# pathint/RankCompV3.jl

Measured on AMD Instinct MI355X. Metric: gene-pair·sample comparisons/sec at 20k genes × 1k samples, higher is better.
Workload: dtype u16

## Files before the change

### rankcompv3.jl_amd/_ffi.py

```python
from __future__ import annotations

import ctypes
import os
import subprocess
from typing import NamedTuple

import numpy as np

_HERE = os.path.dirname(os.path.abspath(__file__))
LIB_PATH = os.environ.get("REO_LIB_PATH") or os.path.join(_HERE, "libreo_hip.so")
CSRC = os.path.join(_HERE, "csrc")

REO_OK, REO_EINVAL, REO_EHIP, REO_ECOMM, REO_ENOMEM = 0, -1, -2, -3, -4
NTIMINGS = 12
CALL_BINS = 8192

SYMBOLS = [
    "reo_version", "reo_last_error", "reo_create", "reo_destroy", "reo_trim_memory", "reo_set_shard", "reo_set_allreduce", "reo_set_allgather",
    "reo_create_multi", "reo_comm_unique_id", "reo_comm_init_rank",
    "reo_set_matrix_f64", "reo_set_matrix_i64", "reo_set_matrix_dev_f64", "reo_set_matrix_dev_i64",
    "reo_set_matrix_f32", "reo_set_matrix_i32", "reo_set_matrix_dev_f32", "reo_set_matrix_dev_i32",
    "reo_set_matrix_rm_f64", "reo_set_matrix_rm_i64", "reo_set_matrix_rm_f32", "reo_set_matrix_rm_i32",
    "reo_set_matrix_csc_f64", "reo_set_matrix_csc_i64", "reo_set_matrix_csc_f32", "reo_set_matrix_csc_i32",
    "reo_set_groups", "reo_compute_thresholds", "reo_set_thresholds", "reo_get_thresholds", "reo_threshold",
# ... 1058 lines not shown
        out = np.zeros((cont.shape[0], 5), dtype=np.float64)
        check(self._L.reo_mccullagh(self._h, _ptr(cont), cont.shape[0], _ptr(out)))
        return out

    @staticmethod
    def _pseudobulk_args(cells, order, chunk_ptr):
        order = np.ascontiguousarray(order, dtype=np.int32)
        chunk_ptr = np.ascontiguousarray(chunk_ptr, dtype=np.int32)
        n_out = chunk_ptr.size - 1
        if hasattr(cells, "tocsc"):
            m = cells.tocsc()
            m.sort_indices()
            G, C = m.shape
            isint = np.issubdtype(m.dtype, np.integer)
            val = np.ascontiguousarray(m.data, dtype=np.int64 if isint else np.float64)
            colptr = np.ascontiguousarray(m.indptr, dtype=np.int64)
            rowidx = np.ascontiguousarray(m.indices, dtype=np.int32)
            args = (G, C, _ptr(colptr), _ptr(rowidx), _ptr(val), _ptr(order), order.size, _ptr(chunk_ptr), n_out)
            return "csc", "i64" if isint else "f64", args, G, (m, val, colptr, rowidx, order, chunk_ptr)
        X = np.asarray(cells)
        isint = np.issubdtype(X.dtype, np.integer)
        Xf = np.asfortranarray(X, dtype=np.int64 if isint else np.float64)
        G, C = Xf.shape
        args = (_ptr(Xf), G, C, G, _ptr(order), order.size, _ptr(chunk_ptr), n_out)
        return "dense", "i64" if isint else "f64", args, G, (Xf, order, chunk_ptr)

    def pseudobulk(self, cells, order, chunk_ptr) -> np.ndarray:
        form, ty, args, G, keep = self._pseudobulk_args(cells, order, chunk_ptr)
        out = np.zeros((G, args[-1]), dtype=np.int64 if ty == "i64" else np.float64, order="F")
        check(getattr(self._L, f"reo_pseudobulk_{form}_{ty}")(self._h, *args, _ptr(out)))
        return out

    def set_matrix_pseudobulk(self, cells, order, chunk_ptr) -> None:
        if is_device_sparse(cells) or is_device_tensor(cells):
            order = np.ascontiguousarray(order, dtype=np.int32)
            chunk_ptr = np.ascontiguousarray(chunk_ptr, dtype=np.int32)
            n_out = chunk_ptr.size - 1
            tail = (_ptr(order) if order.size else None, order.size, _ptr(chunk_ptr), n_out)
            if is_device_sparse(cells):
                ty, G, C, nnz, colptr, rowidx, val, bits, keep = device_csc_entry(cells)
                check(getattr(self._L, "reo_set_matrix_pseudobulk_csc_dev_" + ty)(self._h, G, C, nnz, _dptr(colptr), _dptr(rowidx), bits, _dptr(val), *tail))
            else:
                ptr, G, C, ld, ty, keep = device_matrix(cells)
                check(getattr(self._L, "reo_set_matrix_pseudobulk_dense_dev_" + ty)(self._h, ctypes.c_void_p(ptr), G, C, ld, *tail))
            self.G, self.S = G, n_out
            return
        form, ty, args, G, keep = self._pseudobulk_args(cells, order, chunk_ptr)
        check(getattr(self._L, f"reo_set_matrix_pseudobulk_{form}_{ty}")(self._h, *args))
        self.G, self.S = G, args[-1]

    def filter_matrix(self, min_profiles: int = 0, min_features: int = 0):
        info = self.info()
        pk = np.zeros(info["S"], dtype=np.uint8)
        gk = np.zeros(info["G"], dtype=np.uint8)
        sk, gkn = ctypes.c_int64(0), ctypes.c_int64(0)
        check(self._L.reo_filter_matrix(self._h, int(min_profiles), int(min_features), _ptr(pk) if pk.size else None, _ptr(gk) if gk.size else None,
                                        ctypes.byref(sk), ctypes.byref(gkn)))
        self.G, self.S = int(gkn.value), int(sk.value)
        return pk.astype(bool), gk.astype(bool)

    def get_matrix(self) -> np.ndarray:
        info = self.info()
        dt = {1: np.float64, 2: np.int64, 3: np.float32}.get(info["resident_dtype"])
        if dt is None:
            raise DimensionMismatch(REO_EINVAL, "no expression matrix set")
        out = np.zeros((info["G"], info["S"]), dtype=dt, order="F")
        check(self._L.reo_get_matrix(self._h, _ptr(out), out.nbytes))
        return out

    def set_profiling(self, on: bool) -> None:
        check(self._L.reo_set_profiling(self._h, 1 if on else 0))

    def reset_timings(self) -> None:
        check(self._L.reo_reset_timings(self._h))

    def timings(self) -> dict:
        ms = np.zeros(NTIMINGS, dtype=np.float64)
        check(self._L.reo_get_timings(self._h, _ptr(ms), NTIMINGS))
        return {"transform_ms": ms[0], "k1_ms": ms[1], "k2_ms": ms[2], "iter_ms": ms[3], "k3_ms": max(ms[3] - ms[2], 0.0), "k2_launches": int(ms[4]),
                "k1_launches": int(ms[5]), "exchange_ms": ms[6], "pseudobulk_ms": ms[7], "k2_full_ms": ms[8],
                "k2_full_launches": int(ms[9]), "k2_delta_ms": ms[10], "set_matrix_host_wall_ms": ms[11]}

    def info(self) -> dict:
        w = np.zeros(40, dtype=np.int64)
        check(self._L.reo_get_info(self._h, _ptr(w), 40))
        v = np.zeros(28, dtype=np.int64)
        v[:] = w[:28]
        return {"G": int(v[0]), "S": int(v[1]), "Gp": int(v[2]), "table_bytes": int(v[3]), "has_ties": int(v[4]),
                "tiles_owned": int(v[5]), "tiles_total": int(v[6]), "tile_i": int(v[7]), "chunk_j": int(v[8]),
                "chunks_per_panel": int(v[9]), "unit_h": int(v[10]), "sample_slots": int(v[11]),
                "shared_group_counts": int(v[12]), "group_count_bytes": int(v[13]), "transform_in_lds": int(v[14]), "xcc_local_histograms": int(v[15]),
                "cycle_period": int(v[16]), "cycle_found_at_pass": int(v[17]), "cycle_passes_skipped": int(v[18]), "upload_link_bytes": int(v[19]),
                "eager_range_launches": int(v[20]), "rowmajor_upload": int(v[21]),
                "csc_upload": int(v[22]), "csc_nnz": int(v[23]), "resident_dtype": int(v[24]),
                "k1_slot_order": int(v[25]), "k1_half_tiles_separated": int(v[26]), "csc_device": int(v[27]),
                "k1_unslot_form": int(w[28]), "contrast_treat": int(w[29]), "k1_slot_sides": int(w[30]),
                "masked_build": int(w[31]), "k1_slot_slice": int(w[32]), "planes_on_demand": int(w[33]),
                "perm_batch": int(w[34]), "perm_kernel_us": int(w[35]),
                "top_pairs_hist_us": int(w[36]), "top_pairs_emit_us": int(w[37]),
                "top_pairs_null_batch": int(w[38]), "top_pairs_null_us": int(w[39])}
```

### rankcompv3.jl_amd/csrc/api.hip

```cpp
#include <execinfo.h>
#include <signal.h>
#include <unistd.h>

#include <ctime>
#include <algorithm>
#include <chrono>
#include <cmath>
#include <cstdarg>
#include <cstdio>
#include <cstdlib>
#include <cstring>

#include "reo_internal.h"
#include "contrast.h"
#include "masked_pairs.h"
#include "perm_null.h"
#include "sample_counts.h"
#include "upload_csc.h"

#include <mutex>
#include <unordered_map>

namespace reo {

// ... 228 lines not shown
    static bool done = false;
    if (done) return;
    done = true;
    void *warm[2];
    (void)backtrace(warm, 2);
    struct sigaction sa;
    memset(&sa, 0, sizeof sa);
    sa.sa_handler = segv_backtrace;
    sa.sa_flags = SA_NODEFER;
    sigaction(SIGSEGV, &sa, &g_old_action[0]);
    sigaction(SIGBUS, &sa, &g_old_action[1]);
    sigaction(SIGABRT, &sa, &g_old_action[2]);
}

static double wall_us()
{
    timespec ts;
    clock_gettime(CLOCK_MONOTONIC, &ts);
    return ts.tv_sec * 1e6 + ts.tv_nsec * 1e-3;
}

static void drop_ref_mask(reo_ctx *c, const char *why)
{
    c->ref_slot = -1;
    c->ref_gone = why;
}

int32_t wait_or_drop_table(reo_ctx *c)
{
    const hipError_t e = stream_wait(c);
    if (e == hipSuccess) return REO_OK;
    c->built_k = -1;
    c->table_complete = false;
    drop_ref_mask(c, "a kernel queued on this context failed and the class table was dropped");
    set_error("a kernel queued on this context failed: %s (the class table was dropped: call reo_build_pairs again)", hipGetErrorString(e));
    return REO_EHIP;
}

int32_t use(reo_ctx *c)
{
    if (!c) { set_error("null context"); return REO_EINVAL; }
    REO_HIP_CHECK(hipSetDevice(c->device));
    return REO_OK;
}

int32_t no_multi(reo_ctx *c, const char *what)
{
    if (!c) { set_error("null context"); return REO_EINVAL; }
    if (c->in_multi) {
        set_error("%s is not available on a reo_create_multi context (every device would need the matrix: use one process per GPU, each with its own context)", what);
        return REO_EINVAL;
    }
    return REO_OK;
}

bool mask_in_force(reo_ctx *c)
{
    if (c->vmask_set && (c->vmask_G != c->G || c->vmask_S != c->S)) { c->vmask_set = false; c->vwords_valid = false; }
    return c->vmask_set;
}

int32_t refuse_under_mask(reo_ctx *c, const char *what)
{
    if (!c || !mask_in_force(c)) return REO_OK;
    char msg[320];
    mp_query_refusal(what, msg, sizeof msg);
    set_error("%s", msg);
    return REO_EINVAL;
}

static void invalidate(reo_ctx *c)
{
    drop_ref_mask(c, "the matrix or the groups changed after the last reo_identify_degs (reo_set_matrix_*, reo_filter_matrix, reo_set_groups): "
                     "the class table it ran on is gone");
    c->transformed = false;
    c->planes_ready = false; c->planes_on_demand = 0; c->last_k1_slot_slice = 0;
    c->built_k = -1;
    c->built_treat = -1;
    c->built_masked = 0;
    c->gc_valid = false;
    c->eager_k1 = false;
    c->vwords_valid = false;
    (void)mask_in_force(c);
    c->last_k1_slots = 0; c->last_k1_slot_sides = 0; c->k1_slot_items = nullptr; c->k1_slot_items_n = 0; c->k1_slot_gp = 0;
}

static size_t elem_bytes(int dtype) { return dtype >= 3 ? 4 : 8; }

static int32_t check_shape(int64_t G, int64_t S)
{
    if (G < 2 || G > kMaxGenes || S < 2 || S > (1 << 20)) {
        set_error("matrix is %lld x %lld; G must be in [2, %d] and S in [2, 1048576]", (long long)G, (long long)S, kMaxGenes);
        return REO_EINVAL;
    }
    return REO_OK;
}

static int32_t set_matrix(reo_ctx *c, const void *X, int64_t G, int64_t S, int64_t ld, int dtype, bool on_device, int layout = kLayoutColMajor)
{
    const bool rowmajor = layout == kLayoutRowMajor;
    int32_t rc = use(c);
    if (rc) return rc;
    if (dtype >= 3 && getenv("REO_TRANSFORM") && getenv("REO_TRANSFORM")[0] == 's') {
        set_error("REO_TRANSFORM=segmented: the segmented sort of the A/B build takes Float64 and Int64 matrices only, not Float32 / Int32");
        return REO_EINVAL;
    }
    if (!X) { set_error("matrix pointer is null"); return REO_EINVAL; }
    if ((rc = check_shape(G, S))) return rc;
    if (rowmajor && ld < S) { set_error("row pitch %lld < S = %lld (row-major: ld counts the elements from one gene's row to the next)", (long long)ld, (long long)S); return REO_EINVAL; }
    if (layout == kLayoutColMajor && ld < G) { set_error("leading dimension %lld < G = %lld", (long long)ld, (long long)G); return REO_EINVAL; }
    invalidate(c);
    c->rowmajor_upload = 0;
    c->csc_upload = 0; c->csc_nnz = 0; c->csc_device = 0;
    const bool host_i32 = dtype == 4 && !on_device;
    const size_t resident = static_cast<size_t>(G) * S * (dtype == 3 ? 4 : 8);
    c->G = G; c->S = S; c->dtype = dtype == 4 ? 2 : dtype;
    if (on_device && dtype == 4) {
        if ((rc = c->dX_owned.ensure(resident))) return rc;
        c->dX = c->dX_owned.p; c->ld = G;
        if ((rc = widen_device_i32(c, X, ld, G, S, c->dX_owned.p))) { invalidate(c); c->dtype = 0; return rc; }
        if (hipStreamSynchronize(c->stream) != hipSuccess) { set_error("widening the Int32 matrix failed"); invalidate(c); c->dtype = 0; return REO_EHIP; }
    } else if (on_device) {
        c->dX = X; c->ld = ld;
        c->dX_owned.release();
    } else {
        if ((rc = c->dX_owned.ensure(resident))) return rc;
        c->dX = c->dX_owned.p; c->ld = G;
        const bool lds_ranking = G <= 65535 && !(getenv("REO_TRANSFORM") && getenv("REO_TRANSFORM")[0] == 's');
        if (c->eager_mode > 0 && lds_ranking && static_cast<int64_t>(c->group_id.size()) == S && !c->in_multi) {
            const bool k1 = c->eager_mode > 1 && c->ngroups == 2 && c->thr_set && c->world <= 1 && !c->comm && !c->ag && !c->ar && c->k1_wave &&
                            S <= 65535 && !c->k1_stamps;
            c->Gp = static_cast<int>((c->G + kGenePad - 1) / kGenePad) * kGenePad;
            c->Wp = c->Gp / 32;
            if ((rc = c->table.ensure(static_cast<size_t>(c->G) * kPlanes * c->Wp))) return rc;
            const double w0 = wall_us();
            struct DrainUp {
                reo_ctx *c;
                ~DrainUp() { if (c->up) (void)hipStreamSynchronize(c->up); if (c->rk) (void)hipStreamSynchronize(c->rk); }
            } drain_up{c};
            DrainOnExit drain(c);
            rc = eager_upload(c, X, ld, k1, host_i32, layout);
            if (rc) { invalidate(c); return rc; }
            c->rowmajor_upload = rowmajor ? 1 : 0;
            c->csc_upload = layout == kLayoutCsc ? 1 : 0;
            drain.dismiss();
            c->t_ms[11] += (wall_us() - w0) * 1e-3;
            if (c->eager_k1) { c->built_k = 0; c->table_complete = true; }
            return REO_OK;
        }
        struct DrainUp2 {
            reo_ctx *c;
            ~DrainUp2() { if (c->up) (void)hipStreamSynchronize(c->up); }
        } drain_up{c};
        DrainOnExit drain(c);
        const double w0 = wall_us();
        if ((rc = upload_columns(c, X, ld, G, S, c->dX_owned.p, dtype, layout))) { invalidate(c); return rc; }
        c->rowmajor_upload = rowmajor ? 1 : 0;
        c->csc_upload = layout == kLayoutCsc ? 1 : 0;
        drain.dismiss();
        c->t_ms[11] += (wall_us() - w0) * 1e-3;
    }
    return REO_OK;
}

int32_t ensure_transform(reo_ctx *c)
{
    if (c->dtype == 0) { set_error("no expression matrix set"); return REO_EINVAL; }
// ... 118 lines not shown
    c->sc_slot2col_uploaded = c->sc_slot2col.p;
    return REO_OK;
}

int32_t need_complete_table(reo_ctx *c)
{
    if (c->built_k < 0) { set_error("no class table: call reo_build_pairs first"); return REO_EINVAL; }
    if (!c->table_complete) {
        set_error("shard %d of %d holds only its own part of the class table: attach a communicator (reo_comm_init_rank) or an "
                  "exchange hook (reo_set_allgather, reo_set_allreduce) before reo_build_pairs", c->rank, c->world);
        return REO_ECOMM;
    }
    return REO_OK;
}

}

using namespace reo;

extern "C" {

int32_t reo_version(void) { return 1400; }

int32_t reo_trim_memory(void)
{
    std::vector<Block> all;
    {
        Pool &P = pool();
        std::lock_guard<std::mutex> lk(P.mu);
        all.swap(P.free_blocks);
        P.cached = 0;
    }
    int dev = 0;
    const bool have_dev = hipGetDevice(&dev) == hipSuccess;
    for (const Block &b : all) {
        if (!b.pinned) (void)hipSetDevice(b.device);
        raw_free(b.p, b.pinned);
    }
    {
        Handles &H = handles();
        std::lock_guard<std::mutex> lk(H.mu);
        for (int k = 0; k < 2; ++k) {
            for (auto &st : H.streams[k]) { (void)hipSetDevice(st.first); (void)hipStreamDestroy(st.second); }
            for (auto &ev : H.events[k]) { (void)hipSetDevice(ev.first); (void)hipEventDestroy(ev.second); }
            H.streams[k].clear(); H.events[k].clear();
        }
    }
    if (have_dev) (void)hipSetDevice(dev);
    return REO_OK;
}

const char *reo_last_error(void) { return g_err.c_str(); }

int32_t reo_create(reo_ctx **out, int32_t device, uint64_t seed)
{
    if (!out) { set_error("out is null"); return REO_EINVAL; }
    *out = nullptr;
    if (getenv("REO_DEBUG_SEGV")) install_segv_backtrace();
    int ndev = 0;
    if (hipGetDeviceCount(&ndev) != hipSuccess || ndev == 0) {
        set_error("no HIP device visible: libreo_hip has no CPU fallback");
        return REO_EHIP;
    }
    if (device < 0) REO_HIP_CHECK(hipGetDevice(&device));
    if (device >= ndev) { set_error("device %d out of range (%d visible)", device, ndev); return REO_EINVAL; }
    hipDeviceProp_t prop;
    REO_HIP_CHECK(hipGetDeviceProperties(&prop, device));
    if (strncmp(prop.gcnArchName, "gfx950", 6) != 0) {
        set_error("device %d is %s; this library carries gfx950 (MI355X) code objects only", device, prop.gcnArchName);
        return REO_EHIP;
    }
    REO_HIP_CHECK(hipSetDevice(device));
    reo_ctx *c = new (std::nothrow) reo_ctx();
    if (!c) { set_error("out of host memory"); return REO_ENOMEM; }
    c->device = device;
    c->seed = seed;
    if (const char *e = getenv("REO_K1_WAVE")) c->k1_wave = (e[0] != '0');
    if (const char *e = getenv("REO_K1_HALF")) c->k1_half = (e[0] != '0');
    if (const char *e = getenv("REO_K1_SLOTS")) c->k1_slots = (e[0] != '0');
    if (const char *e = getenv("REO_K1_QUEUE")) c->k1_queue = (e[0] != '0');
    if (const char *e = getenv("REO_K1_UNSLOT")) { const int v = atoi(e); c->k1_unslot = (v == 8 || v == 4) ? v : (e[0] == '0' ? 0 : -1); }
    if (const char *e = getenv("REO_K1_SLOT_SIDES")) { const int v = atoi(e); c->k1_slot_sides = (v == 1 || v == 2) ? v : 0; }
    if (const char *e = getenv("REO_K1_SLOT_SLICE")) c->k1_slot_slice = atoi(e) != 0;
    if (const char *e = getenv("REO_K1_WORKERS")) c->k1_workers = std::max(1, atoi(e));
    if (const char *e = getenv("REO_K1_ORDER")) c->k1_order = std::max(0, std::min(2, atoi(e)));
    {
        int n = 0;
        if (hipDeviceGetAttribute(&n, hipDeviceAttributeMultiprocessorCount, c->device) == hipSuccess && n > 0) c->n_cus = n;
    }
    if (const char *e = getenv("REO_SPIN_WAIT")) c->spin_wait = (e[0] != '0');
    if (const char *e = getenv("REO_CHECK_HOOK_TABLE")) c->check_hook_table = (e[0] != '0');
    if (const char *e = getenv("REO_SHARE_GROUP_COUNTS")) c->share_counts = (e[0] != '0');
    if (const char *e = getenv("REO_LIGHT_BAND")) c->light_band = std::max(0, atoi(e));
    if (const char *e = getenv("REO_HIST_BELOW")) c->hist_below = std::max(0, atoi(e));
    if (const char *e = getenv("REO_CYCLE")) c->cycle_watch = atoi(e) != 0;
    if (const char *e = getenv("REO_LIGHT")) c->light_mode = e[0] == '0' ? 0 : (e[0] == '2' ? 2 : (e[0] == '3' ? 3 : 1));
    c->light_window = light_window(); c->light_min_g = light_min_genes();
    if (const char *e = getenv("REO_LIGHT_WINDOW")) c->light_window = std::max(1, std::min(31, atoi(e)));
    if (const char *e = getenv("REO_LIGHT_MIN_G")) c->light_min_g = std::max(64, atoi(e));
    if (const char *e = getenv("REO_STATE_MIRROR")) c->state_mirror_wanted = (e[0] != '0');
    if (const char *e = getenv("REO_EXCHANGE_WAVES")) c->x_waves = std::max(1, std::min(8, atoi(e)));
    if (const char *e = getenv("REO_EAGER_UPLOAD")) c->eager_mode = std::max(0, std::min(2, atoi(e)));
    if (const char *e = getenv("REO_EAGER_CHUNK")) c->eager_chunk = std::max(1, atoi(e));
    if (const char *e = getenv("REO_EAGER_GATE")) c->eager_gate = atoi(e) != 0;
    if (const char *e = getenv("REO_EAGER_RANGES")) c->eager_ranges = std::max(1, std::min(6, atoi(e)));
    if (const char *e = getenv("REO_UPLOAD_THREADS")) c->upload_threads = std::max(0, std::min(64, atoi(e)));
    c->debug_passes = getenv("REO_DEBUG_PASSES") != nullptr;
    c->debug_stamps = getenv("REO_DEBUG_STAMPS") != nullptr;
    c->k1_stamps = getenv("REO_K1_STAMPS") != nullptr;
    hipError_t e = handle_stream(&c->stream, 0);
    if (e != hipSuccess) { delete c; set_error("hipStreamCreate failed: %s", hipGetErrorString(e)); return REO_EHIP; }
    int ok = 0;
    const char *xe = getenv("REO_XCC_LOCAL");
    if (!(xe && xe[0] == '0')) {
        const int32_t rc = xcc_selftest(c, &ok);
        if (rc) { reo_destroy(c); return rc; }
    }
    c->xcc_local = ok;
    *out = c;
    return REO_OK;
}

void reo_destroy(reo_ctx *c)
{
    if (!c) return;
    for (reo_ctx *p : c->peers) reo_destroy(p);
    c->peers.clear();
    (void)hipSetDevice(c->device);
    for (int q = 0; q < 2; ++q) if (c->k1s[q]) (void)hipStreamSynchronize(c->k1s[q]);
    if (c->xs) (void)hipStreamSynchronize(c->xs);
    if (c->up) (void)hipStreamSynchronize(c->up);
    if (c->rk) (void)hipStreamSynchronize(c->rk);
    (void)hipStreamSynchronize(c->stream);
    comm_release(c);
    collect_timings(c);
    tl_release_synced = true;
    for (auto &t : c->pool) { release_event(t.a, 1); release_event(t.b, 1); }
    c->dX_owned.release(); c->pos.release(); c->lo.release(); c->hi.release(); c->goff_dev.release();
    c->table.release();
    c->t_kin.release(); c->t_kout.release(); c->t_vin.release(); c->t_vout.release(); c->t_temp.release();
    c->t_order.release(); c->t_flags.release(); c->t_slots.release(); c->unit_map.release();
    for (auto &il : c->k1_wave_items) il.buf.release();
    for (int q = 0; q < 2; ++q) { release_stream(c->k1s[q], 0); release_event(c->ev_k1_join[q], 0); }
    release_stream(c->xs, 0);
    release_stream(c->up, 0);
    release_stream(c->rk, 1);
    for (auto &e : c->ev_rk) release_event(e, 0);
    for (auto &e : c->ev_up) release_event(e, 0);
    c->e_lists.release();
    for (int q = 0; q < 3; ++q) {
        if (c->stage_h[q]) pool_free(c->stage_h[q], c->stage_cap, true);
        c->stage_d[q].release();
        release_event(c->ev_stage[q], 0);
        release_event(c->ev_widen[q], 0);
    }
    release_event(c->ev_fork, 0);
    release_event(c->ev_x, 0);
    for (auto &e : c->ev_k1) release_event(e, 0);
    c->t_pos16.release(); c->t_lo16.release(); c->t_hi16.release(); c->gcounts.release();
    c->k1_slot_part.release(); c->k1_slot_maps.release(); c->pos_s.release(); c->lo_s.release(); c->k1_queue_ctr.release();
    c->t_pos32.release(); c->t_lo32.release(); c->t_hi32.release(); c->t_vin32.release(); c->t_vout32.release();
    for (int t = 0; t < 2; ++t) { c->refbits[t].release(); c->refbytes[t].release(); }
    c->raw.release(); c->delta_list.release(); c->cont.release(); c->result.release(); c->sorted_d.release(); c->sorted_p.release();
    c->rank_s.release(); c->rank_a.release(); c->scal.release(); c->blockmin.release();
    c->state.release(); c->trace.release(); c->modes.release(); c->cand.release(); c->hist.release(); c->mrank.release(); c->lstate.release(); c->clist.release(); c->olist.release(); c->units_all.release(); c->xsend.release(); c->xrecv.release(); c->check_flag.release(); c->gridbar.release(); c->chunk_v.release(); c->chunk_i.release(); c->part.release();
    if (c->host_state) pool_free(c->host_state, sizeof(IterState), true);
// ... 408 lines not shown
    dg.release(); de.release();
    return rc;
}


static MpState mp_state(reo_ctx *c)
{
    MpState st{};
    st.multi = c->in_multi || !c->peers.empty();
    st.world = c->world;
    st.G = c->dtype ? c->G : 0; st.S = c->dtype ? c->S : 0;
    st.ngroups = c->ngroups;
    st.has_mask = mask_in_force(c);
    return st;
}

static int32_t ensure_valid_words(reo_ctx *c, const char *what)
{
    if (c->vwords_valid && c->vwords.p) return REO_OK;
    std::vector<int32_t> map;
    if (!sc_slot_map(c->group_id.data(), c->S, c->ngroups, map) || c->goff32.empty() || static_cast<int64_t>(map.size()) != c->goff32.back()) {
        set_error("%s: the sample slots of the bit planes do not match the group labels", what);
        return REO_EHIP;
    }
    int32_t rc;
    if ((rc = c->sc_slot2col.ensure(map.size())) || (rc = c->vwords.ensure(map.size() / 32 * static_cast<size_t>(c->Gp)))) return rc;
    if ((rc = upload_slot2col(c, map)) || (rc = launch_valid_words(c, c->sc_slot2col.p))) return rc;
    c->vwords_valid = true;
    return REO_OK;
}

int32_t reo_set_valid_mask(reo_ctx *c, const uint8_t *valid, int64_t G, int64_t S, int64_t ld)
{
    int32_t rc = use(c);
    if (rc) return rc;
    if (!valid) { c->vmask_set = false; c->vwords_valid = false; return REO_OK; }
    char msg[320];
    if (mp_check_mask_args(mp_state(c), G, S, ld, msg, sizeof msg)) { set_error("%s", msg); return REO_EINVAL; }
    REO_HIP_CHECK(stream_wait(c));
    if ((rc = c->vmask.ensure(static_cast<size_t>(G) * S))) { c->vmask_set = false; c->vwords_valid = false; return rc; }
    c->vmask_set = false; c->vwords_valid = false;
    DrainOnExit drain(c);
    REO_HIP_CHECK(hipMemcpy2DAsync(c->vmask.p, static_cast<size_t>(G), valid, static_cast<size_t>(ld), static_cast<size_t>(G), static_cast<size_t>(S),
                                   hipMemcpyHostToDevice, c->stream));
    REO_HIP_CHECK(hipStreamSynchronize(c->stream));
    drain.dismiss();
    c->vmask_set = true; c->vmask_G = G; c->vmask_S = S;
    return REO_OK;
}

int32_t reo_build_pairs_masked(reo_ctx *c, int32_t k, double pval_reo, const int32_t *min_complete)
{
    int32_t rc = use(c);
    if (rc) return rc;
    const MpState st = mp_state(c);
    if (!st.multi && st.world <= 1 && (c->dtype == 0 || c->group_id.empty() || static_cast<int64_t>(c->group_id.size()) != c->S))
        return ensure_transform(c);
    char msg[320];
    if (mp_check_build_args(st, k, pval_reo, min_complete, msg, sizeof msg)) { set_error("%s", msg); return REO_EINVAL; }
    int32_t n1 = 0;
    for (int32_t g : c->group_id) n1 += g == k;
    const int32_t n2 = static_cast<int32_t>(c->S) - n1;
    if (c->mp_thr_n[0] != n1 || c->mp_thr_n[1] != n2 || c->mp_thr_pval != pval_reo || c->mp_thr_host.size() != static_cast<size_t>(n1) + n2 + 2) {
        std::vector<int32_t> m1, m2;
        if (!mp_threshold_table(n1, pval_reo, m1) || !mp_threshold_table(n2, pval_reo, m2)) {
            set_error("reo_build_pairs_masked: no count in 0..n/2 has a two-sided binomial p above %g (the reference's findfirst returns nothing)", pval_reo);
            return REO_EINVAL;
        }
        c->mp_thr_host = m1;
        c->mp_thr_host.insert(c->mp_thr_host.end(), m2.begin(), m2.end());
        c->mp_thr_n[0] = n1; c->mp_thr_n[1] = n2; c->mp_thr_pval = pval_reo;
        c->mp_thr_uploaded = nullptr;
    }
    if ((rc = ensure_transform(c))) return rc;
    if ((rc = c->table.ensure(static_cast<size_t>(c->G) * kPlanes * c->Wp)) || (rc = c->mp_thr.ensure(c->mp_thr_host.size()))) return rc;
    if (c->mp_thr_uploaded != c->mp_thr.p) {
        REO_HIP_CHECK(hipMemcpyAsync(c->mp_thr.p, c->mp_thr_host.data(), c->mp_thr_host.size() * sizeof(int32_t), hipMemcpyHostToDevice, c->stream));
        REO_HIP_CHECK(hipStreamSynchronize(c->stream));
        c->mp_thr_uploaded = c->mp_thr.p;
    }
    if ((rc = ensure_valid_words(c, "reo_build_pairs_masked"))) return rc;
    drop_ref_mask(c, "reo_build_pairs_masked has replaced the class table that the last reo_identify_degs ran on: no reo_identify_degs has run on the current one");
    c->built_k = -1; c->built_treat = -1; c->built_masked = 0; c->eager_k1 = false; c->table_complete = false;
    c->last_k1_slots = 0; c->last_k1_slot_sides = 0; c->k1_slot_items = nullptr; c->k1_slot_items_n = 0; c->k1_slot_gp = 0; c->last_k1_shared = 0;
    REO_HIP_CHECK(hipMemsetAsync(c->table.p, 0, static_cast<size_t>(c->G) * kPlanes * c->Wp * sizeof(uint32_t), c->stream));
    c->table_prezeroed = false;
    if ((rc = launch_pairs_masked(c, k, c->mp_thr.p, n1, c->mp_thr.p + n1 + 1, n2, min_complete[0], min_complete[1]))) return rc;
    c->built_k = k; c->built_masked = 1; c->table_complete = true;
    return REO_OK;
}

int32_t reo_pair_counts_masked(reo_ctx *c, int64_t i0, int64_t i1, int64_t j0, int64_t j1, int32_t *n_gt, int32_t *n_eq, int32_t *n_avail)
{
    int32_t rc = use(c);
    if (rc) return rc;
    const MpState st = mp_state(c);
    if (!st.multi && st.world <= 1 && (c->dtype == 0 || c->group_id.empty() || static_cast<int64_t>(c->group_id.size()) != c->S))
        return ensure_transform(c);
    char msg[320];
    if (mp_check_counts_args(st, i0, i1, j0, j1, n_gt, n_eq, n_avail, msg, sizeof msg)) { set_error("%s", msg); return REO_EINVAL; }
    if ((rc = ensure_transform(c)) || (rc = ensure_valid_words(c, "reo_pair_counts_masked"))) return rc;
    const size_t n = static_cast<size_t>(i1 - i0) * (j1 - j0) * c->ngroups;
    DevBuf<int32_t> dg, de, da;
    if ((rc = dg.ensure(n)) || (rc = de.ensure(n)) || (rc = da.ensure(n))) return rc;
    DrainOnExit drain(c);
    if ((rc = launch_counts_masked(c, i0, i1, j0, j1, dg.p, de.p, da.p))) return rc;
    REO_HIP_CHECK(hipMemcpyAsync(n_gt, dg.p, n * sizeof(int32_t), hipMemcpyDeviceToHost, c->stream));
    REO_HIP_CHECK(hipMemcpyAsync(n_eq, de.p, n * sizeof(int32_t), hipMemcpyDeviceToHost, c->stream));
    REO_HIP_CHECK(hipMemcpyAsync(n_avail, da.p, n * sizeof(int32_t), hipMemcpyDeviceToHost, c->stream));
    if ((rc = wait_or_drop_table(c))) return rc;
    drain.dismiss();
    return REO_OK;
}

int32_t reo_get_codes(reo_ctx *c, int64_t i0, int64_t i1, int64_t j0, int64_t j1, uint8_t *code)
{
    int32_t rc = use(c);
    if (rc) return rc;
    if (c->built_k < 0) { set_error("no class table: call reo_build_pairs first"); return REO_EINVAL; }
    if (!code || i0 < 0 || j0 < 0 || i1 > c->G || j1 > c->G || i0 >= i1 || j0 >= j1) {
        set_error("bad pair block"); return REO_EINVAL;
    }
    const size_t n = static_cast<size_t>(i1 - i0) * (j1 - j0);
    DevBuf<uint8_t> d;
    if ((rc = d.ensure(n))) return rc;
    DrainOnExit drain(c);
    rc = launch_decode(c, i0, i1, j0, j1, d.p);
    if (!rc) {
        hipError_t e = hipMemcpyAsync(code, d.p, n, hipMemcpyDeviceToHost, c->stream);
        if (e == hipSuccess) e = hipStreamSynchronize(c->stream);
        if (e != hipSuccess) { set_error("copy-back failed: %s", hipGetErrorString(e)); rc = REO_EHIP; }
    }
    d.release();
    return rc;
}

int32_t reo_tally(reo_ctx *c, const uint8_t *ref_mask, int32_t *cont)
{
    int32_t rc = use(c);
    if (rc) return rc;
    if ((rc = need_complete_table(c))) return rc;
    if (!ref_mask || !cont) { set_error("null argument"); return REO_EINVAL; }
    if ((rc = ensure_iter_buffers(c))) return rc;
    drop_ref_mask(c, "reo_tally has run since the last reo_identify_degs: it uploads its own mask into the iteration's buffers");
    DrainOnExit drain(c);
    int32_t nref = 0;
    if ((rc = upload_ref(c, ref_mask, 0, &nref))) return rc;
    if ((rc = init_state(c, nref))) return rc;
    if ((rc = launch_tally(c, nref))) return rc;
    REO_HIP_CHECK(hipMemcpyAsync(cont, c->cont.p, sizeof(int32_t) * 9 * c->G, hipMemcpyDeviceToHost, c->stream));
    REO_HIP_CHECK(hipStreamSynchronize(c->stream));
    drain.dismiss();
    collect_timings(c);
    return REO_OK;
}

int32_t reo_identify_degs(reo_ctx *c, const uint8_t *ref0, double pval_deg, double padj_deg, int32_t n_iter,
                          int32_t n_conv, double *result, int32_t *iters_run, int32_t *trace)
{
    int32_t rc = use(c);
    if (rc) return rc;
    drop_ref_mask(c, "the last reo_identify_degs on this context failed");
    if ((rc = need_complete_table(c))) return rc;
    if (!ref0 || !result) { set_error("null argument"); return REO_EINVAL; }
    if ((rc = ensure_iter_buffers(c))) return rc;
    const int64_t G = c->G;
    const int64_t a = static_cast<int64_t>(std::nearbyint(static_cast<double>(G) * 0.05));
    const int64_t b = static_cast<int64_t>(std::nearbyint(static_cast<double>(G) * 0.95));
    if (n_iter > 0 && (a < 1 || b > G || b - a + 1 < 2)) {
// ... 308 lines not shown
        if ((rc = launch_perm_words(c, d_side.p, np, c->sc_slot2col.p, d_aw.p, d_live.p))) return rc;
        REO_HIP_CHECK(hipEventRecord(ev[0], c->stream));
        if ((rc = launch_pairs_permuted(c, d_aw.p, d_live.p, np, n1, static_cast<int>(S) - n1, c->thr[2 * k], c->thr[2 * k + 1], d_tables.p))) return rc;
        REO_HIP_CHECK(hipEventRecord(ev[1], c->stream));
        for (int q = 0; q < np; ++q) {
            const int64_t p = p0 + q;
            loan.lend(d_tables.p + static_cast<size_t>(q) * table_words);
            rc = reo_identify_degs(c, ref_mask, pval_deg, padj_deg, 1, 0, host_res.data(), &iters, nullptr);
            loan.back();
            if (rc) return rc;
            if (q == 0) {
                float ms = 0.f;
                REO_HIP_CHECK(hipEventElapsedTime(&ms, ev[0], ev[1]));
                c->perm_kernel_us += static_cast<int64_t>(ms * 1000.0f + 0.5f);
            }
            if ((rc = launch_perm_accumulate(c, d_obs.p, pval_deg, padj_deg, d_nge.p, d_cnt.p + p, d_cnt.p + n_perm + p, d_se.p + p))) return rc;
            if (delta1_null) memcpy(delta1_null + p * G, host_res.data() + 11 * G, sizeof(double) * G);
        }
    }
    REO_HIP_CHECK(hipMemcpyAsync(n_ge, d_nge.p, sizeof(int32_t) * G, hipMemcpyDeviceToHost, c->stream));
    REO_HIP_CHECK(hipMemcpyAsync(n_up, d_cnt.p, sizeof(int32_t) * n_perm, hipMemcpyDeviceToHost, c->stream));
    REO_HIP_CHECK(hipMemcpyAsync(n_down, d_cnt.p + n_perm, sizeof(int32_t) * n_perm, hipMemcpyDeviceToHost, c->stream));
    REO_HIP_CHECK(hipMemcpyAsync(se_null, d_se.p, sizeof(double) * n_perm, hipMemcpyDeviceToHost, c->stream));
    if ((rc = wait_or_drop_table(c))) return rc;
    drain.dismiss();
    drop_ref_mask(c, "reo_perm_null has run since the last reo_identify_degs: its passes use the iteration's buffers");
    return REO_OK;
}

int32_t reo_mccullagh(reo_ctx *c, const int32_t *cont, int64_t n, double *out)
{
    int32_t rc = use(c);
    if (rc) return rc;
    if (!cont || !out || n < 1) { set_error("bad argument"); return REO_EINVAL; }
    DevBuf<int32_t> dc;
    DevBuf<double> dout;
    if ((rc = dc.ensure(n * 9)) || (rc = dout.ensure(n * 5))) return rc;
    DrainOnExit drain(c);
    hipError_t e = hipMemcpyAsync(dc.p, cont, sizeof(int32_t) * 9 * n, hipMemcpyHostToDevice, c->stream);
    if (e == hipSuccess) {
        rc = launch_mccullagh(c, dc.p, n, dout.p);
        if (!rc) {
            e = hipMemcpyAsync(out, dout.p, sizeof(double) * 5 * n, hipMemcpyDeviceToHost, c->stream);
            if (e == hipSuccess) e = hipStreamSynchronize(c->stream);
        }
    }
    if (e != hipSuccess) { set_error("HIP failure: %s", hipGetErrorString(e)); rc = REO_EHIP; }
    dc.release(); dout.release();
    return rc;
}

int32_t reo_set_profiling(reo_ctx *c, int32_t on)
{
    if (!c) { set_error("null context"); return REO_EINVAL; }
    c->profiling = on != 0;
    for (reo_ctx *p : c->peers) p->profiling = c->profiling;
    return REO_OK;
}

int32_t reo_reset_timings(reo_ctx *c)
{
    if (!c) { set_error("null context"); return REO_EINVAL; }
    collect_timings(c);
    for (double &v : c->t_ms) v = 0.0;
    return REO_OK;
}

int32_t reo_get_timings(reo_ctx *c, double *ms, int32_t n)
{
    if (!c || !ms) { set_error("null argument"); return REO_EINVAL; }
    collect_timings(c);
    for (int i = 0; i < n && i < REO_NTIMINGS; ++i) ms[i] = c->t_ms[i];
    return REO_OK;
}

int32_t reo_get_info(reo_ctx *c, int64_t *info, int32_t n)
{
    if (!c || !info) { set_error("null argument"); return REO_EINVAL; }
    int64_t separated = 0;
    if (n > 26 && c->last_k1_slots) {
        int32_t rc = use(c);
        if (rc || (rc = launch_slot_separated(c, &separated))) return rc;
    }
    const int64_t v[40] = {c->G, c->S, c->Gp, static_cast<int64_t>(c->table.n * sizeof(uint32_t)), c->has_ties,
                           c->tiles_owned, c->tiles_total, kTileI, c->k1_cj, c->k1_q, kUnitH,
                           c->goff32.empty() ? 0 : c->goff32.back(), c->last_k1_shared,
                           static_cast<int64_t>(c->gcounts.n * sizeof(uint16_t)), c->transform_in_lds, c->xcc_local,
                           c->it_cycle_period, c->it_cycle_at, c->it_cycle_skipped, c->narrowed_bytes, c->eager_range_launches, c->rowmajor_upload,
                           c->csc_upload, c->csc_nnz, c->dtype, c->last_k1_slots, separated, c->csc_device,
                           c->last_k1_slots ? c->last_k1_unslot : 0, c->built_k >= 0 ? c->built_treat : -1,
                           c->last_k1_slots ? c->last_k1_slot_sides : 0, (c->built_k >= 0 && c->built_masked) ? 1 : 0,
                           c->last_k1_slots ? c->last_k1_slot_slice : 0, c->transformed ? c->planes_on_demand : 0, c->perm_batch, c->perm_kernel_us,
                           c->top_hist_us, c->top_emit_us, c->top_null_batch, c->top_null_us};
    for (int i = 0; i < n && i < 40; ++i) info[i] = v[i];
    return REO_OK;
}

}
```

### rankcompv3.jl_amd/csrc/k1_slots.h

```cpp
#pragma once

#include <cstddef>
#include <cstdint>

#if defined(__HIPCC__) || defined(__CUDACC__)
#define REO_SLOTS_HD __host__ __device__ inline
#else
#define REO_SLOTS_HD inline
#endif

namespace reo {

constexpr int kSlotTile = 32;
constexpr int kSlotChunk = 256;
constexpr uint32_t kSlotNoMin = 0xFFFFu, kSlotNoMax = 0u;

REO_SLOTS_HD uint32_t slot_pack(uint32_t mn, uint32_t mx) { return mn | mx << 16; }
REO_SLOTS_HD uint32_t slot_min(uint32_t w) { return w & 0xFFFFu; }
REO_SLOTS_HD uint32_t slot_max(uint32_t w) { return w >> 16; }
REO_SLOTS_HD uint32_t slot_join(uint32_t a, uint32_t b)
{
    const uint32_t mn = slot_min(a) < slot_min(b) ? slot_min(a) : slot_min(b), mx = slot_max(a) > slot_max(b) ? slot_max(a) : slot_max(b);
    return slot_pack(mn, mx);
}
// ... 128 lines not shown
            w[k] ^= t << j;
            w[k + j] ^= t;
        }
    }
}

template <int R>
REO_SLOTS_HD void unslot_in_word(uint32_t (&m)[4 * R], int w, uint32_t *T)
{
    unslot_transpose<4 * R>(m);
    if (R == kUnslotWide) {
        REO_SLOTS_UNROLL
        for (int b = 0; b < 4 * R; ++b) T[unslot_lds_index(R, 32u * w + b)] = m[b];
    } else {
        REO_SLOTS_UNROLL
        for (int i = 0; i < 4 * R; ++i) T[unslot_lds_index(R, 32u * w + i) >> 1] = m[i];
    }
}

template <int R>
REO_SLOTS_HD void unslot_out_word(uint32_t (&u)[4 * R], const uint32_t (&ks)[32], int wo, const uint32_t *T, int G, int Gp)
{
    if (R == kUnslotWide) {
        REO_SLOTS_UNROLL
        for (int c = 0; c < 32; ++c) {
            const uint32_t k = ks[c] < static_cast<uint32_t>(Gp) ? ks[c] : static_cast<uint32_t>(Gp - 1);
            u[c % (4 * R)] = T[unslot_lds_index(R, k)];
        }
    } else {
        const uint16_t *T16 = reinterpret_cast<const uint16_t *>(T);
        REO_SLOTS_UNROLL
        for (int c = 0; c < 32; ++c) {
            const uint32_t k = ks[c] < static_cast<uint32_t>(Gp) ? ks[c] : static_cast<uint32_t>(Gp - 1);
            const uint32_t e = T16[unslot_lds_index(R, k)];
            if (c < 16) u[c % (4 * R)] = e;
            else u[c % (4 * R)] |= e << 16;
        }
    }
    unslot_transpose<4 * R>(u);
    const int left = G - 32 * wo;
    const uint32_t valid = left >= 32 ? 0xFFFFFFFFu : (left <= 0 ? 0u : (1u << left) - 1u);
    REO_SLOTS_UNROLL
    for (int q = 0; q < 4 * R; ++q) u[q] &= valid;
}

template <int R>
inline void unslot_group_model(uint32_t *table, int r0, int n_rows, int G, int Wp, const uint32_t *g2s, uint32_t *T)
{
    const int nr = n_rows - r0 < R ? n_rows - r0 : R;
    if (nr <= 0) return;
    uint32_t *rows = table + static_cast<size_t>(r0) * 4 * Wp;
    for (int w = 0; w < Wp; ++w) {
        uint32_t m[4 * R];
        for (int q = 0; q < 4 * R; ++q) m[q] = q < 4 * nr ? rows[static_cast<size_t>(q) * Wp + w] : 0u;
        unslot_in_word<R>(m, w, T);
    }
    for (int wo = 0; wo < Wp; ++wo) {
        uint32_t u[4 * R], ks[32];
        for (int c = 0; c < 32; ++c) ks[c] = g2s[32 * wo + c];
        unslot_out_word<R>(u, ks, wo, T, G, 32 * Wp);
        for (int q = 0; q < 4 * nr; ++q) rows[static_cast<size_t>(q) * Wp + wo] = u[q];
    }
}

REO_SLOTS_HD int unslot_pair_bit(int row, int plane) { return 2 * row + plane; }
REO_SLOTS_HD size_t unslot_pair_word(int q, int side, int Wp, int w) { return (static_cast<size_t>(q >> 1) * 4 + 2 * side + (q & 1)) * Wp + w; }

template <int R>
inline void unslot_pair_model(uint32_t *table, int r0, int n_rows, int side, int G, int Wp, const uint32_t *g2s, uint32_t *T)
{
    const int nr = n_rows - r0 < 2 * R ? n_rows - r0 : 2 * R;
    if (nr <= 0) return;
    uint32_t *rows = table + static_cast<size_t>(r0) * 4 * Wp;
    for (int w = 0; w < Wp; ++w) {
        uint32_t m[4 * R];
        for (int q = 0; q < 4 * R; ++q) m[q] = q < 2 * nr ? rows[unslot_pair_word(q, side, Wp, w)] : 0u;
        unslot_in_word<R>(m, w, T);
    }
    for (int wo = 0; wo < Wp; ++wo) {
        uint32_t u[4 * R], ks[32];
        for (int c = 0; c < 32; ++c) ks[c] = g2s[32 * wo + c];
        unslot_out_word<R>(u, ks, wo, T, G, 32 * Wp);
        for (int q = 0; q < 2 * nr; ++q) rows[unslot_pair_word(q, side, Wp, wo)] = u[q];
    }
}

struct alignas(16) SlotQuad { uint32_t x, y, z, w; };

REO_SLOTS_HD int slot_slice_side(int b, int cb, int ce) { return (b >= cb && b < ce) ? 0 : 1; }
REO_SLOTS_HD size_t slot_slice_pos_index(int b, int q, int k, int Gp) { return (static_cast<size_t>(b) * 4 + q) * Gp + k; }
REO_SLOTS_HD size_t slot_slice_rec_index(int b, int k, int Gp) { return (static_cast<size_t>(b) * Gp + k) * 4; }
REO_SLOTS_HD int slot_slice_rec_word(int plane) { return (plane + 15) & 15; }

REO_SLOTS_HD void slot_slice_store(uint32_t (&w)[32], int b, int k0, int k1, int Gp, SlotQuad *Ps, SlotQuad *ALs)
{
    unslot_transpose<32>(w);
    REO_SLOTS_UNROLL
    for (int h = 0; h < 2; ++h) {
        const uint32_t *v = w + 16 * h;
        const int k = h ? k1 : k0;
        REO_SLOTS_UNROLL
        for (int q = 0; q < 4; ++q) Ps[slot_slice_pos_index(b, q, k, Gp)] = SlotQuad{v[4 * q], v[4 * q + 1], v[4 * q + 2], v[4 * q + 3]};
        SlotQuad *r = ALs + slot_slice_rec_index(b, k, Gp);
        r[0] = SlotQuad{v[1], v[2], v[3], v[4]};
        r[1] = SlotQuad{v[5], v[6], v[7], v[8]};
        r[2] = SlotQuad{v[9], v[10], v[11], v[12]};
        r[3] = SlotQuad{v[13], v[14], v[15], v[0]};
    }
}

inline void slot_slice_model(const uint16_t *pos16, const uint32_t *s2g, int Gp, int nblk, int cb, int ce, SlotQuad *Ps, SlotQuad *ALs)
{
    for (int b = 0; b < nblk; ++b) {
        const uint32_t *map = s2g + static_cast<size_t>(slot_slice_side(b, cb, ce)) * Gp;
        for (int k = 0; k < Gp; k += 2) {
            uint32_t w[32];
            for (int s = 0; s < 32; ++s) {
                const uint16_t *row = pos16 + (static_cast<size_t>(b) * 32 + s) * Gp;
                w[s] = static_cast<uint32_t>(row[map[k]]) | static_cast<uint32_t>(row[map[k + 1]]) << 16;
            }
            slot_slice_store(w, b, k, k + 1, Gp, Ps, ALs);
        }
    }
}

inline void slot_slice_scatter_model(const uint16_t *pos16, const uint32_t *g2s, int sides, int Gp, int nblk, int cb, int ce, SlotQuad *Ps, SlotQuad *ALs)
{
    for (int b = 0; b < nblk; ++b) {
        const uint32_t *map = g2s + static_cast<size_t>(sides == 2 ? slot_slice_side(b, cb, ce) : 0) * Gp;
        for (int g = 0; g < Gp; g += 2) {
            uint32_t w[32];
            for (int s = 0; s < 32; ++s) {
                const uint16_t *row = pos16 + (static_cast<size_t>(b) * 32 + s) * Gp;
                w[s] = static_cast<uint32_t>(row[g]) | static_cast<uint32_t>(row[g + 1]) << 16;
            }
            slot_slice_store(w, b, static_cast<int>(map[g]), static_cast<int>(map[g + 1]), Gp, Ps, ALs);
        }
    }
}

inline void slot_permute_row(const uint32_t *in, uint32_t *out, int W, const uint32_t *s2g, int G)
{
    for (int w = 0; w < W; ++w) out[w] = 0;
    for (int k = 0; k < G; ++k) {
        const uint32_t j = s2g[k];
        out[k >> 5] |= ((in[j >> 5] >> (j & 31)) & 1u) << (k & 31);
    }
}

}
```

### rankcompv3.jl_amd/csrc/kernels.hip

```cpp
#include <algorithm>
#include <chrono>
#include <cstddef>
#include <cstdio>
#include <cstdlib>
#include <cstring>
#include <mutex>
#include <type_traits>

#include "reo_internal.h"
#include "k1_items.h"
#include "k1_slots.h"
#include "k1_queue.h"
#include "contrast.h"
#include "tie_coin.h"

namespace reo {

namespace {

template <bool COH, class T>
__device__ __forceinline__ T ldc(const T *p)
{
    if (COH) return __hip_atomic_load(p, __ATOMIC_RELAXED, __HIP_MEMORY_SCOPE_AGENT);
    return *p;
// ... 75 lines not shown
#pragma unroll
        for (int e = 0; e < kPerThread; ++e) {
            sm_lo[buf * kStageQ + threadIdx.x + 256 * e] = sl[e];
            if (TIES) sm_hi[buf * kStageQ + threadIdx.x + 256 * e] = sh[e];
        }
    };
    stage_load(bb);
    __syncthreads();
    stage_store(0);
    __syncthreads();
    int buf = 0;
    for (int b0 = bb; b0 < be; b0 += kStageB) {
        const bool more = b0 + kStageB < be;
        if (more) stage_load(b0 + kStageB);
        const int nb = idle ? 0 : min(kStageB, be - b0);
        for (int s = 0; s < nb; ++s) {
            Planes16 p[RJ];
#pragma unroll
            for (int r = 0; r < RJ; ++r)
#pragma unroll
                for (int q = 0; q < NQ; ++q) p[r].set(q, P[(static_cast<size_t>(b0 + s) * 4 + q) * Gp + jl + 64 * r]);
            const uint4 *al = sm_lo + buf * kStageQ + s * RI * 4;
            const uint4 *ah = sm_hi + buf * kStageQ + s * RI * 4;
#pragma clang loop unroll(full)
            for (int i = 0; i < RI; ++i) {
                Planes16 a, c;
#pragma unroll
                for (int q = 0; q < 4; ++q) {
                    if (q < 3 && 4 * q + 1 > NB - 1) continue;
                    a.set(q, al[i * 4 + q]);
                    if (TIES) c.set(q, ah[i * 4 + q]);
                }
                uint32_t l[4];
                if (TIES) {
                    chains_first(l, p[0].w[0], p[1].w[0], p[0].w[0], p[1].w[0], a.w[a_word(0)], a.w[a_word(0)], c.w[a_word(0)], c.w[a_word(0)]);
#pragma unroll
                    for (int k = 1; k < NB; ++k)
                        chains_next(l, p[0].w[k], p[1].w[k], p[0].w[k], p[1].w[k], a.w[a_word(k)], a.w[a_word(k)], c.w[a_word(k)], c.w[a_word(k)]);
                } else {
                    chains_first(l, p[0].w[0], p[1].w[0], p[RJ - 2].w[0], p[RJ - 1].w[0], a.w[a_word(0)], a.w[a_word(0)], a.w[a_word(0)], a.w[a_word(0)]);
#pragma unroll
                    for (int k = 1; k < NB; ++k)
                        chains_next(l, p[0].w[k], p[1].w[k], p[RJ - 2].w[k], p[RJ - 1].w[k], a.w[a_word(k)], a.w[a_word(k)], a.w[a_word(k)], a.w[a_word(k)]);
                }
#pragma unroll
                for (int ch = 0; ch < 4; ++ch) {
                    uint32_t &dst = TIES ? (ch < 2 ? gt[ch][i >> 1] : ge[ch - 2][i >> 1]) : gt[ch % RJ][i >> 1];
                    if (i & 1) dst += static_cast<uint32_t>(__builtin_popcount(l[ch])) << 16;
                    else dst += static_cast<uint32_t>(__builtin_popcount(l[ch]));
                }
            }
        }
        if (more) stage_store(buf ^ 1);
        __syncthreads();
        buf ^= 1;
    }
}

struct K1Args {
    const uint4 *P;
    const uint4 *AL;
    const uint4 *AH;
    uint32_t *table;
    const uint32_t *unit_map;
    int G, Gp, Wp;
    int cb, ce, tb, te;
    int gc, gt;
    int nc, nt;
    int m1, m2;
    uint64_t seed;
    int n_units, Q;
    const int32_t *goff;
    int ngroups;
    const uint32_t *items;
    unsigned long long *stamps;
    const int32_t *gate;
    uint32_t *park;
    int32_t *park_ge;
    int park_mode;
    const uint32_t *s2g;
    const uint32_t *trng, *crng;
    uint32_t *queue;
    uint32_t n_items;
};
constexpr size_t kParkSlot = 2 * 64 * 64;

template <int RJ>
__device__ __forceinline__ bool wave_idle(int jw, int i0, int G)
{
    return jw >= G || ((jw + 64 * RJ - 1) >> 6) < (i0 >> 6);
}

__device__ __forceinline__ void shift_in(uint32_t &w, unsigned long long mask)
{
    unsigned long long carry_out;
    asm("v_addc_co_u32 %0, %1, %0, %0, %2" : "+v"(w), "=s"(carry_out) : "s"(mask));
}

__device__ __forceinline__ void write_lane(uint32_t &v, uint32_t x, int l)
{
    asm("v_writelane_b32 %0, %1, %2" : "+v"(v) : "s"(x), "i"(l));
}

template <int RI, int NEAR, typename F>
__device__ __forceinline__ void emit_rows(bool near, int d, unsigned long long lanes_ok, int hi_thr, int lo_thr, uint32_t &wL, uint32_t &wH,
                                          uint32_t &fLlo, uint32_t &fLhi, uint32_t &fHlo, uint32_t &fHhi, F val)
{
#pragma unroll
    for (int ii = RI - 1; ii >= 0; --ii) {
        const int n = val(ii);
        const unsigned long long ok = (NEAR == 1 || (NEAR == 2 && near)) ? (__ballot(d > ii) & lanes_ok) : lanes_ok;
        const unsigned long long mH = __ballot(n >= hi_thr) & ok;
        const unsigned long long mL = __ballot(n <= lo_thr) & ok & ~mH;
        shift_in(wH, mH);
        shift_in(wL, mL);
        write_lane(fHlo, static_cast<uint32_t>(mH), ii);
        write_lane(fHhi, static_cast<uint32_t>(mH >> 32), ii);
        write_lane(fLlo, static_cast<uint32_t>(mL), ii);
        write_lane(fLhi, static_cast<uint32_t>(mL >> 32), ii);
    }
}

template <int RI, bool SPLIT, bool SLOTS = false, typename F>
__device__ __forceinline__ void emit_gene(const K1Args &a, int i0, int j, int bi, int lane, int pl, int hi_thr, int lo_thr, F val)
{
    const int bj = __builtin_amdgcn_readfirstlane(j >> 6);
    if ((bj << 6) >= a.Gp || bj < bi) return;
    const int d = j - i0;
    const bool near = (bj << 6) - i0 < RI;
    const unsigned long long lanes_ok = __ballot(j < a.G);
    uint32_t wL = 0, wH = 0;
    uint32_t fLlo = 0, fLhi = 0, fHlo = 0, fHhi = 0;
    if (!SPLIT) emit_rows<RI, 2>(near, d, lanes_ok, hi_thr, lo_thr, wL, wH, fLlo, fLhi, fHlo, fHhi, val);
    else if (near) emit_rows<RI, 1>(near, d, lanes_ok, hi_thr, lo_thr, wL, wH, fLlo, fLhi, fHlo, fHhi, val);
    else emit_rows<RI, 0>(near, d, lanes_ok, hi_thr, lo_thr, wL, wH, fLlo, fLhi, fHlo, fHhi, val);
    const bool diag = (bj == bi);
    if (lane < RI && i0 + lane < a.G) {
        const size_t gi = SLOTS ? a.s2g[(pl >> 1) * a.Gp + i0 + lane] : static_cast<size_t>(i0 + lane);
        uint32_t *row = a.table + (gi * kPlanes + pl) * a.Wp + 2 * bj;
        if (!diag) {
            *reinterpret_cast<uint2 *>(row) = uint2{fLlo, fLhi};
            *reinterpret_cast<uint2 *>(row + a.Wp) = uint2{fHlo, fHhi};
        } else {
            if (fLlo) atomicOr(row, fLlo);
            if (fLhi) atomicOr(row + 1, fLhi);
            if (fHlo) atomicOr(row + a.Wp, fHlo);
            if (fHhi) atomicOr(row + a.Wp + 1, fHhi);
        }
    }
    if (j < a.G) {
        const size_t gj = SLOTS ? a.s2g[(pl >> 1) * a.Gp + j] : static_cast<size_t>(j);
        uint32_t *row = a.table + (gj * kPlanes + pl) * a.Wp + (i0 >> 5);
        if (RI == 16) {
            const int half = (i0 >> 4) & 1;
            if (!diag) {
                reinterpret_cast<uint16_t *>(row)[half] = static_cast<uint16_t>(wH);
                reinterpret_cast<uint16_t *>(row + a.Wp)[half] = static_cast<uint16_t>(wL);
            } else {
                if (wH) atomicOr(row, wH << (16 * half));
                if (wL) atomicOr(row + a.Wp, wL << (16 * half));
            }
        } else if (!diag) {
            row[0] = wH; row[a.Wp] = wL;
        } else {
            if (wH) atomicOr(row, wH);
            if (wL) atomicOr(row + a.Wp, wL);
// ... 74 lines not shown
    constexpr int RI = kTileI, RJ = TIES ? kRJTies : kRJ;
    int i0, jl;
    if (!tile_of_block<RI, RJ>(a, i0, jl)) return;
    const int lane = threadIdx.x & 63, bi = i0 >> 6;
    __shared__ uint4 sm_lo[2 * kStageB * RI * 4];
    __shared__ uint4 sm_hi[TIES ? 2 * kStageB * RI * 4 : 1];
    const bool idle = wave_idle<RJ>(jl & ~63, i0, a.G);
    uint32_t gt[RJ][RI / 2], ge[TIES ? RJ : 1][RI / 2];

    count_pass<RJ, NB, TIES>(a.P, a.AL, a.AH, a.Gp, i0, jl, a.cb, a.ce, gt, ge, sm_lo, sm_hi, idle);
    emit_side<RI, RJ>(a, i0, jl, bi, lane, 0, a.m1, a.nc - a.m1,
                      [&](int r, int ii) { return count_with_coins<RJ, TIES>(gt, ge, a.seed, i0, jl, r, ii, a.gc); });
    if (!MULTI) {
        count_pass<RJ, NB, TIES>(a.P, a.AL, a.AH, a.Gp, i0, jl, a.tb, a.te, gt, ge, sm_lo, sm_hi, idle);
        emit_side<RI, RJ>(a, i0, jl, bi, lane, 2, a.m2, a.nt - a.m2,
                          [&](int r, int ii) { return count_with_coins<RJ, TIES>(gt, ge, a.seed, i0, jl, r, ii, a.gt); });
    } else {
        uint32_t tot[RJ][RI / 2];
#pragma unroll
        for (int r = 0; r < RJ; ++r)
#pragma unroll
            for (int h = 0; h < RI / 2; ++h) tot[r][h] = 0;
        for (int g = 0; g < a.ngroups; ++g) {
            if (g == a.gc) continue;
            count_pass<RJ, NB, TIES>(a.P, a.AL, a.AH, a.Gp, i0, jl, a.goff[g], a.goff[g + 1], gt, ge, sm_lo, sm_hi, idle);
#pragma unroll
            for (int r = 0; r < RJ; ++r)
#pragma unroll
                for (int h = 0; h < RI / 2; ++h) {
                    if (TIES) {
                        const uint32_t n0 = count_with_coins<RJ, TIES>(gt, ge, a.seed, i0, jl, r, 2 * h, g);
                        const uint32_t n1 = count_with_coins<RJ, TIES>(gt, ge, a.seed, i0, jl, r, 2 * h + 1, g);
                        tot[r][h] += n0 | (n1 << 16);
                    } else tot[r][h] += gt[r][h];
                }
        }
        emit_side<RI, RJ>(a, i0, jl, bi, lane, 2, a.m2, a.nt - a.m2, [&](int r, int ii) { return static_cast<int>(unpack16(tot[r], ii)); });
    }
}


#include "k1_loop_gen.inc"

template <int NB>
__device__ __forceinline__ void k1_loop(u32x16 &c0, u32x16 &c1, u32x16 &c2, u32x16 &c3, const void *pb, uint32_t ps, const void *ab,
                                        uint32_t as, uint32_t nblk, uint32_t poff, uint32_t aoff, uint32_t lds)
{
    if (NB == 12) k1_loop_nb12_free(c0, c1, c2, c3, pb, ps, ab, ab, as, nblk, poff, aoff, lds);
    else if (NB == 15) k1_loop_nb15_free(c0, c1, c2, c3, pb, ps, ab, ab, as, nblk, poff, aoff, lds);
    else if (NB == 16) k1_loop_nb16_free(c0, c1, c2, c3, pb, ps, ab, ab, as, nblk, poff, aoff, lds);
    else if (NB == 17) k1_loop_nb17_free(c0, c1, c2, c3, pb, ps, ab, ab, as, nblk, poff, aoff, lds);
    else k1_loop_nb18_free(c0, c1, c2, c3, pb, ps, ab, ab, as, nblk, poff, aoff, lds);
}

template <int NB>
__device__ __forceinline__ void k1_loop(u32x8 &c0, u32x8 &c1, u32x8 &c2, u32x8 &c3, const void *pb, uint32_t ps, const void *ab,
                                        uint32_t as, uint32_t nblk, uint32_t poff, uint32_t aoff, uint32_t lds)
{
    if (NB == 12) k1_loop_nb12_free_h(c0, c1, c2, c3, pb, ps, ab, ab, as, nblk, poff, aoff, lds);
    else if (NB == 15) k1_loop_nb15_free_h(c0, c1, c2, c3, pb, ps, ab, ab, as, nblk, poff, aoff, lds);
    else if (NB == 16) k1_loop_nb16_free_h(c0, c1, c2, c3, pb, ps, ab, ab, as, nblk, poff, aoff, lds);
    else if (NB == 17) k1_loop_nb17_free_h(c0, c1, c2, c3, pb, ps, ab, ab, as, nblk, poff, aoff, lds);
    else k1_loop_nb18_free_h(c0, c1, c2, c3, pb, ps, ab, ab, as, nblk, poff, aoff, lds);
}

template <int NB, bool TIES, int RI, bool SLOTS = false>
__device__ __forceinline__ void k1w_item(const K1Args &a, uint4 *ring, uint32_t idx, int i0, int jw, int side, unsigned long long t_begin)
{
    constexpr int RJ = kRJ, NE = TIES ? 2 : 1;
    constexpr bool BIG = NB > 16;
    constexpr int LQ = BIG ? 5 : 4, ROWB = BIG ? 128 : 64;
    typedef typename std::conditional<RI == 32, u32x16, u32x8>::type Counts;
    const int lane = threadIdx.x, jl = jw + lane, bi = i0 >> 6;
    const int bb = side ? a.tb : a.cb, be = side ? a.te : a.ce;
    Counts gt0, gt1, gt2, gt3;
    constexpr bool PARK_REGS = NB > 16;
    uint32_t park[(TIES && !PARK_REGS) ? RJ * (RI / 2) : 1];
    Counts ge0 = 0, ge1 = 0, ge2 = 0, ge3 = 0;
    unsigned long long t_loop = 0, t_emit = 0;
    if (a.stamps) t_loop = __builtin_amdgcn_s_memrealtime();
    int sep = 0;
    if constexpr (SLOTS) sep = __builtin_amdgcn_readfirstlane(slot_separated(a.trng[side * (a.Gp >> 5) + (i0 >> 5)], a.crng[side * (a.Gp >> 8) + (jw >> 8)]));
    if (SLOTS && sep) {
        emit_constant<RI>(a, i0, jl, side, sep > 0 ? (side ? a.nt : a.nc) : 0);
    } else if (be > bb) {
        const char *pb = reinterpret_cast<const char *>(a.P) + static_cast<size_t>(bb) * LQ * a.Gp * 16;
        const size_t aoff = (static_cast<size_t>(bb) * a.Gp + i0) * ROWB;
        const uint32_t lds = static_cast<uint32_t>(reinterpret_cast<uintptr_t>(ring));
#pragma clang loop unroll(disable)
        for (int e = 0; e < NE; ++e) {
            const char *ab = reinterpret_cast<const char *>(e ? a.AL : (TIES ? a.AH : a.AL)) + aoff;
            k1_loop<NB>(gt0, gt1, gt2, gt3, pb, static_cast<uint32_t>(a.Gp) * 16u, ab, static_cast<uint32_t>(a.Gp) * static_cast<uint32_t>(ROWB),
                        static_cast<uint32_t>(be - bb), static_cast<uint32_t>(jl) * 16u, static_cast<uint32_t>(lane) * 16u, lds);
            if (TIES && e == 0) {
                if constexpr (PARK_REGS) { ge0 = gt0; ge1 = gt1; ge2 = gt2; ge3 = gt3; }
                else {
                    constexpr int W = (TIES && !PARK_REGS) ? RI / 2 : 0;
#pragma unroll
                    for (int h = 0; h < W; ++h) { park[h] = gt0[h]; park[W + h] = gt1[h]; park[2 * W + h] = gt2[h]; park[3 * W + h] = gt3[h]; }
                }
            }
        }
    } else {
        gt0 = 0; gt1 = 0; gt2 = 0; gt3 = 0;
#pragma unroll
        for (int h = 0; h < ((TIES && !PARK_REGS) ? RJ * (RI / 2) : 1); ++h) park[h] = 0;
    }
    if (a.stamps) t_emit = __builtin_amdgcn_s_memrealtime();
    if (!SLOTS && a.park_mode) {
        constexpr int W4 = RI / 8;
        uint4 *slot = reinterpret_cast<uint4 *>(a.park + static_cast<size_t>(idx) * kParkSlot) + lane;
        auto add4 = [&](Counts &v, const uint4 *p) {
#pragma unroll
            for (int q = 0; q < W4; ++q) { const uint4 w = p[q * 64]; v[4 * q] += w.x; v[4 * q + 1] += w.y; v[4 * q + 2] += w.z; v[4 * q + 3] += w.w; }
        };
        auto put4 = [&](const Counts &v, uint4 *p) {
#pragma unroll
            for (int q = 0; q < W4; ++q) p[q * 64] = uint4{v[4 * q], v[4 * q + 1], v[4 * q + 2], v[4 * q + 3]};
        };
        if (a.park_mode & 1) {
            const uint4 *ge_from = slot + ((TIES && __builtin_amdgcn_readfirstlane(a.park_ge[idx])) ? 4 * W4 * 64 : 0);
            if constexpr (TIES && PARK_REGS) { add4(ge0, ge_from); add4(ge1, ge_from + W4 * 64); add4(ge2, ge_from + 2 * W4 * 64); add4(ge3, ge_from + 3 * W4 * 64); }
            else if constexpr (TIES) {
#pragma clang loop unroll(disable)
                for (int cq = 0; cq < 4 * W4; ++cq) { const uint4 w = ge_from[cq * 64]; park[4 * cq] += w.x; park[4 * cq + 1] += w.y; park[4 * cq + 2] += w.z; park[4 * cq + 3] += w.w; }
            }
            add4(gt0, slot); add4(gt1, slot + W4 * 64); add4(gt2, slot + 2 * W4 * 64); add4(gt3, slot + 3 * W4 * 64);
        }
        if (a.park_mode & 2) {
            put4(gt0, slot); put4(gt1, slot + W4 * 64); put4(gt2, slot + 2 * W4 * 64); put4(gt3, slot + 3 * W4 * 64);
            if constexpr (TIES && PARK_REGS) { uint4 *ge_to = slot + 4 * W4 * 64; put4(ge0, ge_to); put4(ge1, ge_to + W4 * 64); put4(ge2, ge_to + 2 * W4 * 64); put4(ge3, ge_to + 3 * W4 * 64); }
            else if constexpr (TIES) {
                uint4 *ge_to = slot + 4 * W4 * 64;
#pragma clang loop unroll(disable)
                for (int cq = 0; cq < 4 * W4; ++cq) ge_to[cq * 64] = uint4{park[4 * cq], park[4 * cq + 1], park[4 * cq + 2], park[4 * cq + 3]};
            }
            if (lane == 0) a.park_ge[idx] = TIES ? 1 : 0;
            return;
        }
    }
    const int g = side ? a.gt : a.gc;
    const int m = side ? a.m2 : a.m1, n = side ? a.nt : a.nc;
#pragma clang loop unroll(disable)
    for (int r = 0; r < ((SLOTS && sep) ? 0 : RJ); ++r) {
        const Counts cur = gt0;
        Counts cge = 0;
        if constexpr (TIES && PARK_REGS) cge = ge0;
        else if constexpr (TIES) {
#pragma unroll
            for (int h = 0; h < RI / 2; ++h) cge[h] = park[r * (RI / 2) + h];
        }
        emit_gene<RI, true, SLOTS>(a, i0, jl + 64 * r, bi, lane, side ? 2 : 0, m, n - m, [&](int ii) {
            const uint32_t w = cur[ii >> 1];
            int nre = static_cast<int>((ii & 1) ? (w >> 16) : (w & 0xFFFFu));
            if (TIES) {
                const uint32_t w2 = cge[ii >> 1];
                const int nge = static_cast<int>((ii & 1) ? (w2 >> 16) : (w2 & 0xFFFFu));
                const bool amb = (nre < m && nge >= m) || (nre <= n - m && nge > n - m);
                if (amb) nre += tie_wins(a.seed, i0 + ii, jl + 64 * r, g, static_cast<uint32_t>(nge - nre));
            }
            return nre;
        });
        gt0 = gt1; gt1 = gt2; gt2 = gt3;
        if constexpr (TIES && PARK_REGS) { ge0 = ge1; ge1 = ge2; ge2 = ge3; }
    }
    if (a.stamps && lane == 0) {
        unsigned long long *st = a.stamps + static_cast<size_t>(idx) * 4;
// ... 58 lines not shown

constexpr int kSlotSplits = 16;
constexpr int kSlotRankSpan = 2048;

__global__ __launch_bounds__(256) void k1_slot_part(const uint16_t *__restrict__ pos16, int Gp, int G, int s0a, int na, int s0b, int nb, uint32_t *__restrict__ part)
{
    const int g = blockIdx.x * 256 + threadIdx.x, split = blockIdx.y, side = blockIdx.z;
    if (g >= G) return;
    const int s0 = side ? s0b : s0a, n = side ? nb : na;
    const int per = (n + kSlotSplits - 1) / kSlotSplits;
    const int b = min(n, split * per), e = min(n, b + per);
    uint32_t mn = kSlotNoMin, mx = kSlotNoMax;
#pragma unroll 4
    for (int s = b; s < e; ++s) {
        const uint32_t v = pos16[static_cast<size_t>(s0 + s) * Gp + g];
        mn = min(mn, v); mx = max(mx, v);
    }
    part[(static_cast<size_t>(split) * 2 + side) * Gp + g] = slot_pack(mn, mx);
}

__global__ __launch_bounds__(256) void k1_slot_keys(const uint32_t *__restrict__ part, int Gp, int G, int sides, uint32_t *__restrict__ gmm, uint32_t *__restrict__ key)
{
    const int g = blockIdx.x * 256 + threadIdx.x;
    if (g >= G) return;
    uint32_t r0 = slot_pack(kSlotNoMin, kSlotNoMax), r1 = r0;
#pragma unroll
    for (int y = 0; y < kSlotSplits; ++y) {
        r0 = slot_join(r0, part[(static_cast<size_t>(y) * 2) * Gp + g]);
        r1 = slot_join(r1, part[(static_cast<size_t>(y) * 2 + 1) * Gp + g]);
    }
    gmm[g] = r0; gmm[Gp + g] = r1;
    if (sides == 2) { key[g] = slot_side_key(r0); key[Gp + g] = slot_side_key(r1); }
    else key[g] = slot_key(r0, r1);
}

template <bool K32>
__global__ __launch_bounds__(kSlotRankSpan / 2) void k1_slot_sort(const uint32_t *__restrict__ key, int G, int Gp, void *__restrict__ srt_)
{
    typedef typename std::conditional<K32, uint32_t, uint64_t>::type Key;
    __shared__ Key sk[kSlotRankSpan];
    key += static_cast<size_t>(blockIdx.y) * Gp;
    Key *srt = static_cast<Key *>(srt_) + (static_cast<size_t>(blockIdx.y) * gridDim.x + blockIdx.x) * kSlotRankSpan;
    const int h0 = blockIdx.x * kSlotRankSpan, t = threadIdx.x;
    for (int e = t; e < kSlotRankSpan; e += kSlotRankSpan / 2) {
        Key v = static_cast<Key>(~0ull);
        if (h0 + e < G) {
            if constexpr (K32) v = slot_order_key32(key[h0 + e], static_cast<uint32_t>(h0 + e));
            else v = slot_order_key(key[h0 + e], static_cast<uint32_t>(h0 + e));
        }
        sk[e] = v;
    }
    for (int k = 2; k <= kSlotRankSpan; k <<= 1)
        for (int j = k >> 1; j > 0; j >>= 1) {
            __syncthreads();
            const int l = ((t & ~(j - 1)) << 1) | (t & (j - 1)), r = l | j;
            const Key x = sk[l], y = sk[r];
            if ((x > y) == ((l & k) == 0)) { sk[l] = y; sk[r] = x; }
        }
    __syncthreads();
    for (int e = t; e < kSlotRankSpan; e += kSlotRankSpan / 2) srt[e] = sk[e];
}

template <bool K32>
__global__ __launch_bounds__(256) void k1_slot_rank(const uint32_t *__restrict__ key, const void *__restrict__ srt_, int G, int Gp, uint32_t *__restrict__ g2s)
{
    typedef typename std::conditional<K32, uint32_t, uint64_t>::type Key;
    __shared__ Key sk[kSlotRankSpan];
    key += static_cast<size_t>(blockIdx.z) * Gp; g2s += static_cast<size_t>(blockIdx.z) * Gp;
    const Key *srt = static_cast<const Key *>(srt_) + (static_cast<size_t>(blockIdx.z) * gridDim.y + blockIdx.y) * kSlotRankSpan;
    for (int t = threadIdx.x; t < kSlotRankSpan; t += 256) sk[t] = srt[t];
    __syncthreads();
    const int g = blockIdx.x * 256 + threadIdx.x;
    if (g >= G) return;
    Key mine;
    if constexpr (K32) mine = slot_order_key32(key[g], static_cast<uint32_t>(g));
    else mine = slot_order_key(key[g], static_cast<uint32_t>(g));
    uint32_t n = 0;
#pragma unroll
    for (int step = kSlotRankSpan / 2; step > 0; step >>= 1) n += sk[n + step - 1] < mine ? step : 0;
    n += sk[n] < mine ? 1u : 0u;
    if (n) atomicAdd(&g2s[g], n);
}

__global__ __launch_bounds__(256) void k1_slot_invert(uint32_t *__restrict__ g2s, uint32_t *__restrict__ s2g, int G, int Gp, int sides)
{
    const int g = blockIdx.x * 256 + threadIdx.x;
    if (g >= Gp) return;
    if (sides == 2) { g2s += static_cast<size_t>(blockIdx.y) * Gp; s2g += static_cast<size_t>(blockIdx.y) * Gp; }
    uint32_t k = static_cast<uint32_t>(g), v = static_cast<uint32_t>(g);
    if (g < G) { k = g2s[g]; if (k >= static_cast<uint32_t>(G)) return; }
    else g2s[g] = v;
    s2g[k] = v;
    if (sides != 2) s2g[static_cast<size_t>(Gp) + k] = v;
}

__global__ __launch_bounds__(256) void k1_slot_ranges(const uint32_t *__restrict__ gmm, const uint32_t *__restrict__ s2g, int G, int Gp,
                                                      uint32_t *__restrict__ trng, uint32_t *__restrict__ crng)
{
    static_assert(kSlotTile == kTileI && kSlotChunk == 64 * kRJ, "k1_slots.h carries its own copy of the item geometry");
    __shared__ uint32_t sm[8];
    const int k = blockIdx.x * 256 + threadIdx.x, side = blockIdx.y;
    uint32_t r = k < G ? gmm[static_cast<size_t>(side) * Gp + s2g[static_cast<size_t>(side) * Gp + k]] : slot_pack(kSlotNoMin, kSlotNoMax);
#pragma unroll
    for (int o = 1; o < 32; o <<= 1) r = slot_join(r, static_cast<uint32_t>(__shfl_xor(static_cast<int>(r), o)));
    if ((threadIdx.x & 31) == 0) { trng[static_cast<size_t>(side) * (Gp >> 5) + (k >> 5)] = r; sm[threadIdx.x >> 5] = r; }
    __syncthreads();
    if (threadIdx.x == 0) {
        for (int q = 1; q < 8; ++q) r = slot_join(r, sm[q]);
        crng[static_cast<size_t>(side) * (Gp >> 8) + blockIdx.x] = r;
    }
}

__global__ __launch_bounds__(256) void k1_slot_gather(const uint4 *__restrict__ P, const uint4 *__restrict__ AL, const uint32_t *__restrict__ s2g, int Gp, int cb, int ce,
                                                      uint4 *__restrict__ Ps, uint4 *__restrict__ ALs)
{
    const int k = blockIdx.x * 256 + threadIdx.x, b = blockIdx.y;
    if (b < cb || b >= ce) s2g += Gp;
    const uint32_t g = s2g[k];
#pragma unroll
    for (int q = 0; q < 4; ++q) Ps[(static_cast<size_t>(b) * 4 + q) * Gp + k] = P[(static_cast<size_t>(b) * 4 + q) * Gp + g];
#pragma unroll
    for (int e = 0; e < 4; ++e) {
        const int kk = blockIdx.x * 256 + e * 64 + (threadIdx.x >> 2), q = threadIdx.x & 3;
        ALs[(static_cast<size_t>(b) * Gp + kk) * 4 + q] = AL[(static_cast<size_t>(b) * Gp + s2g[kk]) * 4 + q];
    }
}

__global__ __launch_bounds__(256) void k1_slot_slice(const uint16_t *__restrict__ pos16, const uint32_t *__restrict__ g2s, int map_sides, int Gp, int nblk, int cb, int ce, int per,
                                                     SlotQuad *__restrict__ Ps, SlotQuad *__restrict__ ALs)
{
    const int wpb = Gp >> 9;
    const int v = static_cast<int>(blockIdx.x & 7u) * per + static_cast<int>(blockIdx.x >> 3);
    if (v >= nblk * wpb) return;
    const int b = v / wpb, g = ((v - b * wpb) * 256 + static_cast<int>(threadIdx.x)) * 2;
    const uint2 k2 = *reinterpret_cast<const uint2 *>(g2s + static_cast<size_t>(map_sides == 2 ? slot_slice_side(b, cb, ce) : 0) * Gp + g);
    const int k0 = static_cast<int>(min(k2.x, static_cast<uint32_t>(Gp - 1))), k1 = static_cast<int>(min(k2.y, static_cast<uint32_t>(Gp - 1)));
    const uint32_t *rows2 = reinterpret_cast<const uint32_t *>(pos16 + static_cast<size_t>(b) * 32 * Gp) + (g >> 1);
    uint32_t w[32];
#pragma unroll
    for (int s = 0; s < 32; ++s) w[s] = rows2[static_cast<size_t>(s) * (Gp >> 1)];
    slot_slice_store(w, b, k0, k1, Gp, Ps, ALs);
}

template <int R>
__global__ __launch_bounds__(256) void k1_unslot_columns(uint32_t *__restrict__ table, const uint32_t *__restrict__ g2s, int G, int Wp)
{
    extern __shared__ uint4 unslot_sm[];
    uint32_t *sm = reinterpret_cast<uint32_t *>(unslot_sm);
    const int r0 = blockIdx.x * R, nr = min(R, G - r0);
    if (nr <= 0) return;
    uint32_t *rows = table + static_cast<size_t>(r0) * kPlanes * Wp;
    for (int rp = 0; rp < nr * kPlanes; ++rp)
        for (int w = threadIdx.x; w < Wp; w += 256) sm[(static_cast<size_t>(rp >> 2) * Wp + w) * 4 + (rp & 3)] = rows[static_cast<size_t>(rp) * Wp + w];
    __syncthreads();
    for (int wo = threadIdx.x; wo < Wp; wo += 256) {
        uint32_t acc[R][4];
#pragma unroll
        for (int r = 0; r < R; ++r) acc[r][0] = acc[r][1] = acc[r][2] = acc[r][3] = 0;
        const uint4 *kq = reinterpret_cast<const uint4 *>(g2s) + static_cast<size_t>(wo) * 8;
#pragma unroll 2
        for (int i = 0; i < 8; ++i) {
            const uint4 k4 = kq[i];
            const uint32_t ks[4] = {k4.x, k4.y, k4.z, k4.w};
#pragma unroll
            for (int e = 0; e < 4; ++e) {
                const uint32_t k = ks[e], kw = min(k >> 5, static_cast<uint32_t>(Wp - 1)), kb = k & 31u;
#pragma unroll
                for (int r = 0; r < R; ++r) {
                    if (r < nr) {
                        const uint4 w = unslot_sm[static_cast<size_t>(r) * Wp + kw];
                        acc[r][0] = __builtin_amdgcn_alignbit(w.x >> kb, acc[r][0], 1);
                        acc[r][1] = __builtin_amdgcn_alignbit(w.y >> kb, acc[r][1], 1);
                        acc[r][2] = __builtin_amdgcn_alignbit(w.z >> kb, acc[r][2], 1);
                        acc[r][3] = __builtin_amdgcn_alignbit(w.w >> kb, acc[r][3], 1);
                    }
                }
            }
        }
        const int left = G - 32 * wo;
        const uint32_t valid = left >= 32 ? 0xFFFFFFFFu : (left <= 0 ? 0u : (1u << left) - 1u);
#pragma unroll
        for (int r = 0; r < R; ++r)
            if (r < nr) {
#pragma unroll
                for (int pl = 0; pl < 4; ++pl) rows[(static_cast<size_t>(r) * kPlanes + pl) * Wp + wo] = acc[r][pl] & valid;
            }
    }
}

template <int R>
__global__ __launch_bounds__(kUnslotThreadsMax) void k1_unslot_words(uint32_t *__restrict__ table, const uint32_t *__restrict__ g2s, int G, int Wp)
{
    constexpr int NQ = 4 * R;
    extern __shared__ uint32_t unslot_t[];
    const int r0 = blockIdx.x * R, nr = min(R, G - r0);
    if (nr <= 0) return;
    const int nq = nr * kPlanes;
    uint32_t *rows = table + static_cast<size_t>(r0) * kPlanes * Wp;
    for (int w = threadIdx.x; w < Wp; w += blockDim.x) {
        uint32_t m[NQ];
#pragma unroll
        for (int q = 0; q < NQ; ++q) m[q] = q < nq ? rows[static_cast<size_t>(q) * Wp + w] : 0u;
        unslot_in_word<R>(m, w, unslot_t);
    }
    __syncthreads();
    for (int wo = threadIdx.x; wo < Wp; wo += blockDim.x) {
        const uint4 *kq = reinterpret_cast<const uint4 *>(g2s) + static_cast<size_t>(wo) * 8;
        uint32_t ks[32], u[NQ];
#pragma unroll
        for (int i = 0; i < 8; ++i) {
            const uint4 k4 = kq[i];
            ks[4 * i] = k4.x; ks[4 * i + 1] = k4.y; ks[4 * i + 2] = k4.z; ks[4 * i + 3] = k4.w;
        }
        unslot_out_word<R>(u, ks, wo, unslot_t, G, 32 * Wp);
#pragma unroll
        for (int q = 0; q < NQ; ++q)
            if (q < nq) rows[static_cast<size_t>(q) * Wp + wo] = u[q];
    }
}

template <int R>
__global__ __launch_bounds__(kUnslotThreadsMax) void k1_unslot_pair(uint32_t *__restrict__ table, const uint32_t *__restrict__ g2s, int G, int Wp)
{
    constexpr int NQ = 4 * R;
    extern __shared__ uint32_t unslot_t[];
    const int r0 = blockIdx.x * 2 * R, nr = min(2 * R, G - r0), side = blockIdx.y;
    if (nr <= 0) return;
    const int nq = nr * 2;
    g2s += static_cast<size_t>(side) * 32 * Wp;
    uint32_t *rows = table + static_cast<size_t>(r0) * kPlanes * Wp;
    for (int w = threadIdx.x; w < Wp; w += blockDim.x) {
        uint32_t m[NQ];
#pragma unroll
        for (int q = 0; q < NQ; ++q) m[q] = q < nq ? rows[unslot_pair_word(q, side, Wp, w)] : 0u;
        unslot_in_word<R>(m, w, unslot_t);
    }
    __syncthreads();
    for (int wo = threadIdx.x; wo < Wp; wo += blockDim.x) {
        const uint4 *kq = reinterpret_cast<const uint4 *>(g2s) + static_cast<size_t>(wo) * 8;
        uint32_t ks[32], u[NQ];
#pragma unroll
        for (int i = 0; i < 8; ++i) {
            const uint4 k4 = kq[i];
            ks[4 * i] = k4.x; ks[4 * i + 1] = k4.y; ks[4 * i + 2] = k4.z; ks[4 * i + 3] = k4.w;
        }
        unslot_out_word<R>(u, ks, wo, unslot_t, G, 32 * Wp);
#pragma unroll
        for (int q = 0; q < NQ; ++q)
            if (q < nq) rows[unslot_pair_word(q, side, Wp, wo)] = u[q];
    }
}

__global__ __launch_bounds__(256) void k1_slot_count(const uint32_t *__restrict__ items, int n, const uint32_t *__restrict__ trng, const uint32_t *__restrict__ crng,
                                                     int Gp, unsigned long long *__restrict__ out)
{
    const int i = blockIdx.x * 256 + threadIdx.x;
    int v = 0;
    if (i < n) {
        const uint32_t it = items[i];
        const int side = slot_item_side(it);
        if (slot_separated(trng[static_cast<size_t>(side) * (Gp >> 5) + slot_item_tile(it)], crng[static_cast<size_t>(side) * (Gp >> 8) + slot_item_chunk(it)]))
            v = slot_item_halves(it);
    }
    const unsigned long long m1 = __ballot(v == 1), m2 = __ballot(v == 2);
    if ((threadIdx.x & 63) == 0 && (m1 | m2)) atomicAdd(out, static_cast<unsigned long long>(__builtin_popcountll(m1) + 2 * __builtin_popcountll(m2)));
}

template <int NB>
__global__ __launch_bounds__(64, NB > 16 ? 2 : 3) void k1w_pairs_gated(K1Args a)
{
    constexpr int RI = kTileI;
    constexpr int ROWB = NB > 16 ? 128 : 64;
    __shared__ uint4 ring[2 * RI * ROWB / 16];
    const int bad = a.gate[0] | a.gate[4] | a.gate[5], ties = a.gate[1];
    if (bad) return;
    if (ties) k1w_body<NB, true>(a, ring, blockIdx.x);
    else k1w_body<NB, false>(a, ring, blockIdx.x);
}

constexpr int kRJWide = 2, kRJWideTies = 1;

template <int RJ, int NB, bool TIES>
__device__ __forceinline__ void count_pass_wide(const uint4 *__restrict__ P, const uint4 *__restrict__ AL, const uint4 *__restrict__ AH,
                                                int Gp, int i0, int jl, int bb, int be, uint32_t (&gt)[RJ][kTileI],
                                                uint32_t (&ge)[TIES ? RJ : 1][kTileI], uint4 *sm_lo, uint4 *sm_hi, bool idle)
{
    static_assert((TIES && RJ == 1) || (!TIES && RJ == 2), "four chains per bit plane");
    constexpr int RI = kTileI, NQ = (NB + 3) / 4;
    constexpr int kStageQ = kStageB * RI * 4;
    constexpr int kPerThread = kStageQ / 256;
#pragma unroll
    for (int r = 0; r < RJ; ++r)
#pragma unroll
        for (int ii = 0; ii < RI; ++ii) { gt[r][ii] = 0; if (TIES) ge[r][ii] = 0; }
    if (bb >= be) return;
    uint4 sl[kPerThread], sh[TIES ? kPerThread : 1];
    auto stage_load = [&](int b0) {
#pragma unroll
        for (int e = 0; e < kPerThread; ++e) {
            const int idx = threadIdx.x + 256 * e;
            const int b = min(b0 + idx / (RI * 4), be - 1);
            const size_t o = (static_cast<size_t>(b) * Gp + i0) * 4 + idx % (RI * 4);
            sl[e] = AL[o];
            if (TIES) sh[e] = AH[o];
        }
    };
    auto stage_store = [&](int buf) {
#pragma unroll
        for (int e = 0; e < kPerThread; ++e) {
            sm_lo[buf * kStageQ + threadIdx.x + 256 * e] = sl[e];
            if (TIES) sm_hi[buf * kStageQ + threadIdx.x + 256 * e] = sh[e];
        }
    };
    stage_load(bb);
    __syncthreads();
    stage_store(0);
    __syncthreads();
// ... 2750 lines not shown

static void dispatch_pairs(reo_ctx *c, const K1Args &a, const K1Plan &pl)
{
    switch (plane_bits(c->G)) {
    case 12: launch_pairs<12>(c, a, pl); break;
    case 15: launch_pairs<15>(c, a, pl); break;
    case 16: launch_pairs<16>(c, a, pl); break;
    case 17: launch_pairs<17>(c, a, pl); break;
    default: launch_pairs<18>(c, a, pl); break;
    }
}

static int32_t upload_units_all(reo_ctx *c);

struct StoredItems { uint64_t key[7]; std::vector<uint32_t> units, items; };
static std::mutex g_item_store_mu;
static std::vector<StoredItems> *const g_item_store = new std::vector<StoredItems>();

static int32_t item_list(reo_ctx *c, const K1Args &a, const K1Plan &pl, int sides, const std::vector<uint32_t> &units, reo_ctx::ItemList &cache, int part, int nparts)
{
    K1ItemGeom g;
    g.G = static_cast<int>(c->G); g.RJ = pl.RJ; g.CJ = pl.CJ; g.Q = pl.Q;
    g.nsides = pl.wave ? 2u : 1u; g.sides = sides;
    g.wave = pl.wave; g.wide = pl.wide; g.big = pl.big;
    g.halves = pl.wave && !pl.wide && c->k1_half;
    g.side_blocks = pl.wave ? std::max(a.ce - a.cb, a.te - a.tb) : c->goff32[c->ngroups] / 32;
    g.order = c->k1_order; g.n_cus = c->n_cus;
    const uint64_t key[5] = {static_cast<uint64_t>(c->G) << 32 | static_cast<uint32_t>(c->Gp), static_cast<uint64_t>(g.halves ? 1 : 0) << 48 | static_cast<uint64_t>(g.RJ) << 32 | static_cast<uint32_t>(g.Q),
                             static_cast<uint64_t>(c->world) << 32 | static_cast<uint32_t>(c->rank),
                             static_cast<uint64_t>(g.nsides) << 56 | static_cast<uint64_t>(units.size()) << 24 | static_cast<uint64_t>(g.side_blocks),
                             static_cast<uint64_t>(sides) << 48 | static_cast<uint64_t>(part) << 32 | static_cast<uint32_t>(nparts)};
    if (cache.buf.p && std::memcmp(key, cache.key, sizeof key) == 0) return REO_OK;
    const uint64_t skey[7] = {key[0], key[1], key[2], key[3], key[4], static_cast<uint64_t>(c->n_cus),
                              static_cast<uint64_t>(c->k1_order) << 2 | static_cast<uint64_t>(g.big ? 1 : 0) << 1 | static_cast<uint64_t>(g.wide ? 1 : 0)};
    std::vector<uint32_t> items;
    bool have = false;
    {
        std::lock_guard<std::mutex> lk(g_item_store_mu);
        for (const StoredItems &st : *g_item_store)
            if (std::memcmp(st.key, skey, sizeof skey) == 0 && st.units == units) { items = st.items; have = true; break; }
    }
    if (!have) {
        items = k1_item_list(g, units);
        std::lock_guard<std::mutex> lk(g_item_store_mu);
        if (g_item_store->size() >= 16) g_item_store->erase(g_item_store->begin());
        StoredItems st;
        std::memcpy(st.key, skey, sizeof skey);
        st.units = units; st.items = items;
        g_item_store->push_back(std::move(st));
    }
    int32_t rc;
    if ((rc = cache.buf.ensure(std::max<size_t>(items.size(), 1)))) return rc;
    if (!items.empty()) {
        REO_HIP_CHECK(hipMemcpyAsync(cache.buf.p, items.data(), items.size() * sizeof(uint32_t), hipMemcpyHostToDevice, c->stream));
        REO_HIP_CHECK(hipStreamSynchronize(c->stream));
    }
    cache.n = items.size();
    std::memcpy(cache.key, key, sizeof key);
    return REO_OK;
}

template <class F>
static int32_t pipelined_exchange(reo_ctx *c, const K1Args &a, const K1Plan &pl, int nwaves, int maxu_x, F dispatch_wave)
{
    int32_t rc;
    const std::vector<uint32_t> &units = pl.units;
    const int mw = (maxu_x + nwaves - 1) / nwaves;
    const size_t uw = static_cast<size_t>(exchange_unit_words(c));
    if ((rc = c->xsend.ensure(uw * mw * nwaves)) || (rc = c->xrecv.ensure(uw * mw * nwaves * c->world))) return rc;
    if (!c->xs) {
        for (int q = 0; q < 2; ++q) REO_HIP_CHECK(handle_stream(&c->k1s[q], 0));
        REO_HIP_CHECK(handle_stream(&c->xs, 0));
        REO_HIP_CHECK(handle_event(&c->ev_fork, 0));
        REO_HIP_CHECK(handle_event(&c->ev_x, 0));
        for (int q = 0; q < 2; ++q) REO_HIP_CHECK(handle_event(&c->ev_k1_join[q], 0));
        for (int q = 0; q < 8; ++q) REO_HIP_CHECK(handle_event(&c->ev_k1[q], 0));
    }
    std::vector<std::vector<uint32_t>> wunits(nwaves);
    for (size_t m = 0; m < units.size(); ++m) wunits[std::min<size_t>(m / mw, nwaves - 1)].push_back(units[m]);
    for (int w = 0; w < nwaves; ++w)
        if ((rc = item_list(c, a, pl, 3, wunits[w], c->k1_wave_items[w], w, nwaves))) return rc;
    if ((rc = upload_units_all(c))) return rc;
    if (!c->table_prezeroed) REO_HIP_CHECK(hipMemsetAsync(c->table.p, 0, static_cast<size_t>(c->G) * kPlanes * c->Wp * sizeof(uint32_t), c->stream));
    c->table_prezeroed = false;
    c->last_k1_shared = 0;
    tic(c, 1);
    int32_t xrc = REO_OK;
    auto hip_ok = [&](hipError_t e, const char *what) {
        if (e == hipSuccess || xrc) return e == hipSuccess;
        set_error("%s failed: %s (pipelined exchange)", what, hipGetErrorString(e));
        xrc = e == hipErrorOutOfMemory ? REO_ENOMEM : REO_EHIP;
        return false;
    };
    bool forked = hip_ok(hipEventRecord(c->ev_fork, c->stream), "hipEventRecord(fork)");
    for (int q = 0; q < 2 && forked; ++q) forked = hip_ok(hipStreamWaitEvent(c->k1s[q], c->ev_fork, 0), "hipStreamWaitEvent(fork)");
    if (forked) forked = hip_ok(hipStreamWaitEvent(c->xs, c->ev_fork, 0), "hipStreamWaitEvent(fork)");
    for (int w = 0; w < nwaves && !xrc; ++w) {
        hipStream_t ks = c->k1s[w & 1];
        dispatch_wave(w, ks);
        if (!hip_ok(hipGetLastError(), "pair kernel launch")) break;
        if (!hip_ok(hipEventRecord(c->ev_k1[w], ks), "hipEventRecord(wave)") || !hip_ok(hipStreamWaitEvent(c->xs, c->ev_k1[w], 0), "hipStreamWaitEvent(wave)")) break;
        const int m0 = w * mw, mc = std::max(0, std::min(mw, maxu_x - m0));
        if (mc == 0) continue;
        uint32_t *send = c->xsend.p + uw * mw * w, *recv = c->xrecv.p + uw * mw * w * c->world;
        const int64_t bytes = static_cast<int64_t>(uw) * mc * sizeof(uint32_t);
        if ((xrc = launch_pack_units(c, m0, mc, send, c->xs))) break;
        if (c->comm) { if ((xrc = comm_allgather(c, send, recv, bytes, c->xs)) < 0) break; xrc = REO_OK; }
        else {
            const int hrc = c->ag(send, recv, bytes, c->xs, c->ag_user);
            if (hrc) { set_error("all-gather hook failed with %d", hrc); xrc = REO_ECOMM; break; }
        }
        if ((xrc = launch_expand_units(c, m0, mc, recv, c->xs))) break;
    }
    bool joined = true;
    for (int q = 0; q < 2; ++q)
        if (hipEventRecord(c->ev_k1_join[q], c->k1s[q]) != hipSuccess || hipStreamWaitEvent(c->stream, c->ev_k1_join[q], 0) != hipSuccess) joined = false;
    toc(c);
    tic(c, 6);
    if (hipEventRecord(c->ev_x, c->xs) != hipSuccess || hipStreamWaitEvent(c->stream, c->ev_x, 0) != hipSuccess) joined = false;
    toc(c);
    if (!joined) {
        for (int q = 0; q < 2; ++q) (void)hipStreamSynchronize(c->k1s[q]);
        (void)hipStreamSynchronize(c->xs);
        if (!xrc) { set_error("joining the streams of the pipelined exchange failed"); xrc = REO_EHIP; }
    }
    if (xrc) return xrc;
    c->x_pipelined = true;
    return REO_OK;
}

static int32_t report_k1_stamps(reo_ctx *c, unsigned long long *stamps)
{
    std::vector<unsigned long long> h(c->k1_items_n * 4 + 2);
    REO_HIP_CHECK(hipMemcpyAsync(h.data(), stamps, h.size() * sizeof(unsigned long long), hipMemcpyDeviceToHost, c->stream));
    REO_HIP_CHECK(hipStreamSynchronize(c->stream));
    double pro = 0, loop = 0, emit = 0;
    unsigned long long t0 = ~0ull, t1 = 0;
    for (size_t i = 0; i < c->k1_items_n; ++i) {
        pro += static_cast<double>(h[4 * i + 1] - h[4 * i]); loop += static_cast<double>(h[4 * i + 2] - h[4 * i + 1]);
        emit += static_cast<double>(h[4 * i + 3] - h[4 * i + 2]);
        t0 = std::min(t0, h[4 * i]); t1 = std::max(t1, h[4 * i + 3]);
    }
    const double n = static_cast<double>(c->k1_items_n) * 100.0;
    fprintf(stderr, "[reo] K1 wave items %zu: prologue %.2f us, count loop %.2f us, classification %.2f us per item; first start to last end %.3f ms\n",
            c->k1_items_n, pro / n, loop / n, emit / n, static_cast<double>(t1 - t0) / 1e5);
    fprintf(stderr, "[reo]   a launch before it ended %.1f us before the first item began; one after it began %.1f us after the last item ended\n",
            static_cast<double>(static_cast<long long>(t0 - h[c->k1_items_n * 4])) / 100.0, static_cast<double>(static_cast<long long>(h[c->k1_items_n * 4 + 1] - t1)) / 100.0);
    constexpr int kSl = 24;
    const double span = static_cast<double>(t1 - t0) + 1.0;
    double busy[kSl] = {}, dur[kSl] = {};
    size_t started[kSl] = {};
    for (size_t i = 0; i < c->k1_items_n; ++i) {
        const double b = static_cast<double>(h[4 * i] - t0), e = static_cast<double>(h[4 * i + 3] - t0);
        const int s0 = static_cast<int>(b / span * kSl);
        started[s0]++; dur[s0] += static_cast<double>(h[4 * i + 2] - h[4 * i + 1]);
        for (int s = s0; s < kSl; ++s) {
            const double lo = span * s / kSl, hi = span * (s + 1) / kSl;
            if (e <= lo) break;
            busy[s] += (std::min(e, hi) - std::max(b, lo)) / (hi - lo);
        }
    }
    fprintf(stderr, "[reo]   items in flight by slice:");
    for (int s = 0; s < kSl; ++s) fprintf(stderr, " %.0f", busy[s]);
    fprintf(stderr, "\n[reo]   loop us of items started in slice:");
    for (int s = 0; s < kSl; ++s) fprintf(stderr, " %.0f", started[s] ? dur[s] / static_cast<double>(started[s]) / 100.0 : 0.0);
    fprintf(stderr, "\n");
    (void)hipFree(stamps);
    return REO_OK;
}

static K1Args k1_args(const reo_ctx *c, int k)
{
    K1Args a;
    a.P = c->pos.p; a.AL = c->lo.p; a.AH = c->hi.p; a.table = c->table.p;
    a.G = static_cast<int>(c->G); a.Gp = c->Gp; a.Wp = c->Wp;
    const bool multi = c->ngroups > 2;
    const int other = multi ? k : 1 - k;
    a.cb = c->goff32[k] / 32; a.ce = c->goff32[k + 1] / 32;
    a.tb = c->goff32[other] / 32; a.te = c->goff32[other + 1] / 32;
    a.gc = k; a.gt = other;
    a.nc = c->goff[k + 1] - c->goff[k]; a.nt = static_cast<int>(c->S) - a.nc;
    a.goff = c->goff_dev.p; a.ngroups = c->ngroups;
    a.m1 = c->thr[2 * k]; a.m2 = c->thr[2 * k + 1];
    a.seed = c->seed;
    a.items = nullptr; a.stamps = nullptr; a.gate = nullptr;
    a.park = nullptr; a.park_ge = nullptr; a.park_mode = 0;
    a.s2g = nullptr; a.trng = nullptr; a.crng = nullptr;
    a.queue = nullptr; a.n_items = 0;
    return a;
}

static int32_t upload_unit_map(reo_ctx *c, const std::vector<uint32_t> &units)
{
    int32_t rc;
    if ((rc = c->unit_map.ensure(std::max<size_t>(units.size(), 1)))) return rc;
    if (!units.empty() && (c->unit_map.p != c->unit_map_uploaded || units != c->unit_map_host)) {
        REO_HIP_CHECK(hipMemcpyAsync(c->unit_map.p, units.data(), units.size() * sizeof(uint32_t), hipMemcpyHostToDevice, c->stream));
        REO_HIP_CHECK(hipStreamSynchronize(c->stream));
        c->unit_map_host = units;
        c->unit_map_uploaded = c->unit_map.p;
    }
    return REO_OK;
}

static int32_t apply_range(reo_ctx *c, K1Args &a, int sides, const K1Range *range, size_t n_items)
{
    int32_t rc;
    const int side = sides == 1 ? 0 : 1, sb = side ? a.tb : a.cb, se = side ? a.te : a.ce;
    if (range->b0 < 0 || range->b1 <= range->b0 || sb + range->b1 > se || (range->first != (range->b0 == 0)) || (range->last != (sb + range->b1 == se))) {
        set_error("a range of sample blocks outside its side"); return REO_EINVAL;
    }
    if (!(range->first && range->last)) {
        if ((rc = c->k1_park[side].ensure(std::max<size_t>(n_items, 1) * kParkSlot)) || (rc = c->k1_park_ge[side].ensure(std::max<size_t>(n_items, 1)))) return rc;
        a.park = c->k1_park[side].p; a.park_ge = c->k1_park_ge[side].p;
        a.park_mode = (range->first ? 0 : 1) | (range->last ? 0 : 2);
    }
    (side ? a.tb : a.cb) = sb + range->b0;
    (side ? a.te : a.ce) = sb + range->b1;
    return REO_OK;
}


struct SlotMaps { uint32_t *gmm, *key, *g2s, *s2g, *trng, *crng; unsigned long long *count, *srt; };
static size_t slot_maps_words(int Gp) { return static_cast<size_t>(Gp) * 8 + static_cast<size_t>(Gp) / 16 + static_cast<size_t>(Gp) / 128 + 2 + 4 * (static_cast<size_t>(Gp) + kSlotRankSpan); }
static SlotMaps slot_maps(const reo_ctx *c)
{
    SlotMaps m;
    const size_t Gp = static_cast<size_t>(c->Gp);
    m.gmm = c->k1_slot_maps.p; m.key = m.gmm + 2 * Gp; m.g2s = m.key + 2 * Gp; m.s2g = m.g2s + 2 * Gp;
    m.trng = m.s2g + 2 * Gp; m.crng = m.trng + Gp / 16;
    m.count = reinterpret_cast<unsigned long long *>(m.crng + Gp / 128);
    m.srt = m.count + 1;
    return m;
}

static bool k1_slots_wanted(const reo_ctx *c, const K1Plan &pl, int sides, bool keep_table, const int32_t *gate, const K1Range *range, bool prepare)
{
    return c->k1_slots && pl.wave && !pl.wide && !pl.big && c->ngroups == 2 && sides == 3 && !c->has_ties && c->world == 1 && !c->in_multi &&
           !gate && !range && !prepare && !keep_table && c->t_pos16.p && c->t_pos16.n >= static_cast<size_t>(c->goff32[2]) * c->Gp;
}

static int32_t k1_slots_alloc(reo_ctx *c)
{
    int32_t rc;
    const size_t nq = static_cast<size_t>(c->goff32[2] / 32) * c->Gp * 4;
    if ((rc = c->k1_slot_part.ensure(static_cast<size_t>(kSlotSplits) * 2 * c->Gp)) || (rc = c->k1_slot_maps.ensure(slot_maps_words(c->Gp))) ||
        (rc = c->pos_s.ensure(nq)) || (rc = c->lo_s.ensure(nq)))
        return rc;
    if (c->k1_queue && c->k1_queue_ctr.ensure(kQueueWords)) (void)hipGetLastError();
    return REO_OK;
}

static int32_t k1_slots_front(reo_ctx *c, K1Args &a, int sides)
{
    const int G = a.G, Gp = a.Gp, nblk = c->goff32[2] / 32;
    const SlotMaps m = slot_maps(c);
    const unsigned gb = static_cast<unsigned>((G + 255) / 256), zs = static_cast<unsigned>(sides);
    REO_HIP_CHECK(hipMemsetAsync(m.g2s, 0, static_cast<size_t>(Gp) * 4 * sizeof(uint32_t), c->stream));
    k1_slot_part<<<dim3(gb, kSlotSplits, 2), 256, 0, c->stream>>>(c->t_pos16.p, Gp, G, a.cb * 32, a.nc, a.tb * 32, a.nt, c->k1_slot_part.p);
    k1_slot_keys<<<gb, 256, 0, c->stream>>>(c->k1_slot_part.p, Gp, G, sides, m.gmm, m.key);
    const unsigned spans = static_cast<unsigned>((G + kSlotRankSpan - 1) / kSlotRankSpan);
    if (slot_order_key32_fits(G)) {
        k1_slot_sort<true><<<dim3(spans, zs), kSlotRankSpan / 2, 0, c->stream>>>(m.key, G, Gp, m.srt);
        k1_slot_rank<true><<<dim3(gb, spans, zs), 256, 0, c->stream>>>(m.key, m.srt, G, Gp, m.g2s);
    } else {
        k1_slot_sort<false><<<dim3(spans, zs), kSlotRankSpan / 2, 0, c->stream>>>(m.key, G, Gp, m.srt);
        k1_slot_rank<false><<<dim3(gb, spans, zs), 256, 0, c->stream>>>(m.key, m.srt, G, Gp, m.g2s);
    }
    k1_slot_invert<<<dim3(static_cast<unsigned>(Gp / 256), zs), 256, 0, c->stream>>>(m.g2s, m.s2g, G, Gp, sides);
    k1_slot_ranges<<<dim3(static_cast<unsigned>(Gp / 256), 2), 256, 0, c->stream>>>(m.gmm, m.s2g, G, Gp, m.trng, m.crng);
    if (c->k1_slot_slice) {
        const int per = (nblk * (Gp / 512) + 7) / 8;
        SlotQuad *ps = reinterpret_cast<SlotQuad *>(c->pos_s.p), *als = reinterpret_cast<SlotQuad *>(c->lo_s.p);
        k1_slot_slice<<<static_cast<unsigned>(per * 8), 256, 0, c->stream>>>(c->t_pos16.p, m.g2s, sides, Gp, nblk, a.cb, a.ce, per, ps, als);
    } else {
        k1_slot_gather<<<dim3(static_cast<unsigned>(Gp / 256), static_cast<unsigned>(nblk)), 256, 0, c->stream>>>(c->pos.p, c->lo.p, m.s2g, Gp, a.cb, a.ce, c->pos_s.p, c->lo_s.p);
    }
    REO_HIP_CHECK(hipGetLastError());
    c->last_k1_slot_slice = c->k1_slot_slice ? 1 : 0;
    a.P = c->pos_s.p; a.AL = c->lo_s.p; a.AH = c->lo_s.p;
    a.s2g = m.s2g; a.trng = m.trng; a.crng = m.crng;
    a.n_items = static_cast<uint32_t>(c->k1_items_n);
    if (c->k1_queue && c->k1_queue_ctr.p && c->k1_queue_ctr.n >= static_cast<size_t>(kQueueWords)) {
        REO_HIP_CHECK(hipMemsetAsync(c->k1_queue_ctr.p, 0, kQueueWords * sizeof(uint32_t), c->stream));
        a.queue = c->k1_queue_ctr.p;
    }
    return REO_OK;
}

static int32_t k1_slots_back(reo_ctx *c, const K1Args &a, int sides)
{
    if (c->k1_unslot != 0) {
        int form = unslot_form(a.Gp);
        if ((c->k1_unslot == kUnslotWide || c->k1_unslot == kUnslotNarrow) && unslot_lds_bytes(c->k1_unslot, a.Gp) <= kUnslotLdsLimit) form = c->k1_unslot;
        const size_t lds = unslot_lds_bytes(form, a.Gp);
        if (lds <= kUnslotLdsLimit) {
            auto go = [&](auto rtag) -> int32_t {
                constexpr int R = decltype(rtag)::value;
                const int bit = (R == kUnslotWide ? 1 : 2) << (sides == 2 ? 2 : 0);
                const void *fn = sides == 2 ? reinterpret_cast<const void *>(k1_unslot_pair<R>) : reinterpret_cast<const void *>(k1_unslot_words<R>);
                if (!(c->k1_unslot_attr & bit)) {
                    REO_HIP_CHECK(hipFuncSetAttribute(fn, hipFuncAttributeMaxDynamicSharedMemorySize, static_cast<int>(kUnslotLdsLimit)));
                    c->k1_unslot_attr |= bit;
                }
                const unsigned threads = static_cast<unsigned>(unslot_threads(a.Wp));
                if (sides == 2)
                    k1_unslot_pair<R><<<dim3(static_cast<unsigned>((a.G + 2 * R - 1) / (2 * R)), 2), threads, lds, c->stream>>>(a.table, slot_maps(c).g2s, a.G, a.Wp);
                else
                    k1_unslot_words<R><<<static_cast<unsigned>((a.G + R - 1) / R), threads, lds, c->stream>>>(a.table, slot_maps(c).g2s, a.G, a.Wp);
                return REO_OK;
            };
            const int32_t rc = form == kUnslotWide ? go(std::integral_constant<int, kUnslotWide>{}) : go(std::integral_constant<int, kUnslotNarrow>{});
            if (rc) return rc;
            REO_HIP_CHECK(hipGetLastError());
            c->last_k1_unslot = form;
            return REO_OK;
        }
    }
    if (sides != 1) { set_error("the bit form of the column un-permute: the common slot order only"); return REO_EINVAL; }
    c->last_k1_unslot = 1;
    const size_t row_bytes = static_cast<size_t>(a.Wp) * 16;
    auto go = [&](auto rtag) {
        constexpr int R = decltype(rtag)::value;
        k1_unslot_columns<R><<<static_cast<unsigned>((a.G + R - 1) / R), 256, R * row_bytes, c->stream>>>(a.table, slot_maps(c).g2s, a.G, a.Wp);
    };
    if (6 * row_bytes <= 61440) go(std::integral_constant<int, 6>{});
    else if (4 * row_bytes <= 61440) go(std::integral_constant<int, 4>{});
    else if (2 * row_bytes <= 61440) go(std::integral_constant<int, 2>{});
    else go(std::integral_constant<int, 1>{});
    REO_HIP_CHECK(hipGetLastError());
    return REO_OK;
}

int32_t launch_slot_separated(reo_ctx *c, int64_t *half_tiles)
{
    *half_tiles = 0;
    if (!c->last_k1_slots || !c->k1_slot_items || !c->k1_slot_items_n || !c->k1_slot_maps.p) return REO_OK;
    const reo_ctx::ItemList &il = c->k1_wave_items[0];
    if (c->k1_slot_gp != c->Gp || c->k1_slot_maps.n < slot_maps_words(c->Gp) || c->k1_slot_items != il.buf.p || c->k1_slot_items_n > il.buf.n) return REO_OK;
    const SlotMaps m = slot_maps(c);
    unsigned long long n = 0;
    REO_HIP_CHECK(hipMemsetAsync(m.count, 0, sizeof n, c->stream));
    k1_slot_count<<<static_cast<unsigned>((c->k1_slot_items_n + 255) / 256), 256, 0, c->stream>>>(c->k1_slot_items, static_cast<int>(c->k1_slot_items_n), m.trng, m.crng, c->Gp, m.count);
    REO_HIP_CHECK(hipGetLastError());
    REO_HIP_CHECK(hipMemcpyAsync(&n, m.count, sizeof n, hipMemcpyDeviceToHost, c->stream));
    REO_HIP_CHECK(hipStreamSynchronize(c->stream));
    *half_tiles = static_cast<int64_t>(n);
    return REO_OK;
}

int32_t launch_k1(reo_ctx *c, int k, int sides, bool keep_table, const int32_t *gate, const K1Range *range, bool prepare, int treat)
{
    K1Args a = k1_args(c, k);
    K1Plan pl;
    int32_t rc;
    if (treat >= 0) {
        if (sides != 3 || keep_table || gate || range || prepare || c->ngroups <= 2) { set_error("a contrast of two groups: more than two groups, the whole table"); return REO_EINVAL; }
        const ContrastSides cs = contrast_sides(c->goff.data(), c->goff32.data(), c->thr.data(), k, treat);
        a.cb = cs.cb; a.ce = cs.ce; a.tb = cs.tb; a.te = cs.te;
        a.gc = k; a.gt = treat;
        a.nc = cs.nc; a.nt = cs.nt; a.m1 = cs.m1; a.m2 = cs.m2;
        pl.contrast = true;
    }
    if ((rc = k1_plan(c, sides, pl))) return rc;
    const std::vector<uint32_t> &units = pl.units;
    c->units_all_host = pl.units_all;
    c->tiles_owned = pl.tiles_owned; c->tiles_total = pl.tiles_total;
    c->k1_cj = pl.CJ; c->k1_q = pl.Q;
    a.n_units = static_cast<int>(units.size()); a.Q = pl.Q;
    if ((rc = upload_unit_map(c, units))) return rc;
    a.unit_map = c->unit_map.p;
    a.gate = gate;
    if (!prepare) { c->last_k1_slots = 0; c->last_k1_slot_sides = 0; c->last_k1_slot_slice = 0; c->k1_slot_items = nullptr; c->k1_slot_items_n = 0; c->k1_slot_gp = 0; }
    if ((range || prepare) && (sides != 1 && sides != 2)) { set_error("a range of sample blocks / a prepared launch: one side of the pair kernel"); return REO_EINVAL; }
    if (gate && (!pl.wave || pl.wide || pl.big)) { set_error("a gated launch of the pair kernel: wave form, at most 65535 genes and samples"); return REO_EINVAL; }
    c->x_pipelined = false;
    const int maxu_x = exchange_units_per_rank(c);
    const int nwaves = (pl.wave && sides == 3 && c->world > 1 && (c->comm || c->ag) && !c->in_multi && !c->k1_stamps) ? std::min({c->x_waves, 8, maxu_x}) : 1;
    if (nwaves > 1) {
        hipStream_t main_stream = c->stream;
        return pipelined_exchange(c, a, pl, nwaves, maxu_x, [&](int w, hipStream_t ks) {
            c->stream = ks;
            a.items = c->k1_wave_items[w].buf.p; c->k1_items_n = c->k1_wave_items[w].n;
            if (c->k1_items_n) dispatch_pairs(c, a, pl);
            c->stream = main_stream;
        });
    }
    if (pl.wave || (pl.wcounts && !c->gc_valid) || pl.wmulti) {
        reo_ctx::ItemList &il = c->k1_wave_items[sides == 3 ? 0 : sides];
        const auto w0 = std::chrono::steady_clock::now();
        if ((rc = item_list(c, a, pl, sides, units, il, 0, 1))) return rc;
        if (c->debug_passes) fprintf(stderr, "  launch_k1 sides %d: item list (%zu items) ready after %.0f us\n", sides, il.n, std::chrono::duration<double, std::micro>(std::chrono::steady_clock::now() - w0).count());
        a.items = il.buf.p; c->k1_items_n = il.n;
        if (prepare) return REO_OK;
        if (range && (rc = apply_range(c, a, sides, range, il.n))) return rc;
        if (c->k1_stamps) REO_HIP_CHECK(hipMalloc(reinterpret_cast<void **>(&a.stamps), (std::max<size_t>(c->k1_items_n, 1) * 4 + 2) * sizeof(unsigned long long)));
    }
    if (!keep_table) {
        if (!c->table_prezeroed) REO_HIP_CHECK(hipMemsetAsync(c->table.p, 0, static_cast<size_t>(c->G) * kPlanes * c->Wp * sizeof(uint32_t), c->stream));
        c->table_prezeroed = false;
    }
    if (units.empty()) return REO_OK;
    c->last_k1_shared = pl.shared ? 1 : 0;
    if (k1_slots_wanted(c, pl, sides, keep_table, gate, range, prepare) && c->k1_items_n) {
        if (k1_slots_alloc(c) == REO_OK) pl.slots = true;
        else (void)hipGetLastError();
    }
    if (!(pl.slots && c->k1_slot_slice) && (rc = ensure_planes(c))) return rc;
    if (a.stamps) k_time_mark<<<1, 64, 0, c->stream>>>(a.stamps + c->k1_items_n * 4);
    tic(c, 1);
    const int slot_sides = !pl.slots ? 0 : (c->k1_unslot == 0 ? 1 : slot_sides_wanted(a.ce - a.cb, a.te - a.tb, c->k1_slot_sides));
    if (pl.slots && (rc = k1_slots_front(c, a, slot_sides))) { toc(c); return rc; }
    dispatch_pairs(c, a, pl);
    if (pl.slots && (rc = k1_slots_back(c, a, slot_sides))) { toc(c); return rc; }
    toc(c);
    if (pl.slots) {
        c->last_k1_slots = 1; c->last_k1_slot_sides = slot_sides;
        c->k1_slot_items = a.items; c->k1_slot_items_n = c->k1_items_n; c->k1_slot_gp = a.Gp;
    }
    if (a.stamps) k_time_mark<<<1, 64, 0, c->stream>>>(a.stamps + c->k1_items_n * 4 + 1);
    REO_HIP_CHECK(hipGetLastError());
    if (a.stamps) return report_k1_stamps(c, a.stamps);
    return REO_OK;
}


int64_t exchange_unit_words(const reo_ctx *c) { return static_cast<int64_t>(kUnitRows) * kPlanes * (c->k1_q * c->k1_cj / 32); }
int32_t exchange_units_per_rank(const reo_ctx *c)
{
    const int total = static_cast<int>(c->units_all_host.size()), world = std::max(c->world, 1);
    return std::max(1, (total + world - 1) / world);
}

static int32_t upload_units_all(reo_ctx *c)
{
    int32_t rc;
    const size_t total = c->units_all_host.size();
    if ((rc = c->units_all.ensure(std::max<size_t>(total, 1)))) return rc;
    if (total && (c->units_all.p != c->units_all_uploaded || c->units_all_host != c->units_all_dev)) {
        REO_HIP_CHECK(hipMemcpyAsync(c->units_all.p, c->units_all_host.data(), total * sizeof(uint32_t), hipMemcpyHostToDevice, c->stream));
        REO_HIP_CHECK(hipStreamSynchronize(c->stream));
        c->units_all_dev = c->units_all_host;
        c->units_all_uploaded = c->units_all.p;
    }
    return REO_OK;
}

static int32_t exchange_args(reo_ctx *c, XArgs &a, int m0, int mcnt)
{
    const int32_t rc = upload_units_all(c);
    if (rc) return rc;
    a.table = c->table.p; a.units = c->units_all.p;
    a.G = static_cast<int>(c->G); a.Wp = c->Wp; a.Wc = c->k1_q * c->k1_cj / 32;
    a.total = static_cast<int>(c->units_all_host.size()); a.world = std::max(c->world, 1); a.rank = c->rank; a.maxu = exchange_units_per_rank(c);
    a.m0 = m0; a.mcnt = mcnt < 0 ? a.maxu : mcnt;
    return REO_OK;
}

int32_t launch_pack_units(reo_ctx *c, int m0, int mcnt, uint32_t *send, hipStream_t st)
{
    XArgs a;
    int32_t rc = exchange_args(c, a, m0, mcnt);
    if (rc) return rc;
    const size_t uw = static_cast<size_t>(exchange_unit_words(c));
    x_pack<<<dim3(static_cast<unsigned>((uw + 255) / 256), a.mcnt), 256, 0, st ? st : c->stream>>>(a, send ? send : c->xsend.p);
    REO_HIP_CHECK(hipGetLastError());
    return REO_OK;
}

int32_t launch_expand_units(reo_ctx *c, int m0, int mcnt, const uint32_t *recv, hipStream_t st)
{
    XArgs a;
    int32_t rc = exchange_args(c, a, m0, mcnt);
    if (rc) return rc;
    if (a.world < 2) return REO_OK;
    const size_t uw = static_cast<size_t>(exchange_unit_words(c));
    if (!st) st = c->stream;
    if (!recv) recv = c->xrecv.p;
    x_expand_fwd<<<dim3(static_cast<unsigned>((uw + 255) / 256), a.mcnt * a.world), 256, 0, st>>>(a, recv);
    x_expand_mirror<<<dim3(a.Wc, kPlanes, a.mcnt * a.world), 256, 0, st>>>(a, recv);
    REO_HIP_CHECK(hipGetLastError());
    return REO_OK;
}

int32_t launch_counts(reo_ctx *c, int64_t i0, int64_t i1, int64_t j0, int64_t j1, uint16_t *d_gt, uint16_t *d_eq)
{
    const int32_t rc = ensure_planes(c);
    if (rc) return rc;
    dim3 grid(static_cast<unsigned>((j1 - j0 + 255) / 256), static_cast<unsigned>(i1 - i0));
    if (c->G > 65535)
// ... 223 lines not shown
```

### rankcompv3.jl_amd/csrc/reo_internal.h

```cpp
#pragma once

#include <hip/hip_runtime.h>

#include <cstdint>
#include <functional>
#include <string>
#include <vector>

#include "reo_hip.h"

namespace reo {

constexpr int kTileJ = 256;
constexpr int kTileI = 32;
constexpr int kPlanes = 4;
constexpr int kUnitH = 32;
constexpr int kRJ = 4;
constexpr int kRJTies = 2;
constexpr int kMaxGenes = 262143;
constexpr int kGenePad = 1024;
constexpr int kRaw = 8;
constexpr int kDeltaMax = 128;
constexpr int kSortChunk = 1024;

// ... 135 lines not shown
    reo::DevBuf<unsigned char> dX_owned;
    std::vector<int32_t> group_id;
    int ngroups = 0;
    std::vector<int32_t> thr;
    bool thr_set = false;

    int Gp = 0, Wp = 0;
    std::vector<int32_t> goff;
    std::vector<int32_t> goff32;
    reo::DevBuf<uint4> pos;
    reo::DevBuf<uint4> lo;
    reo::DevBuf<uint4> hi;
    reo::DevBuf<uint16_t> t_pos16, t_lo16, t_hi16;
    reo::DevBuf<uint32_t> t_pos32, t_lo32, t_hi32;
    reo::DevBuf<uint32_t> t_vin32, t_vout32;
    reo::DevBuf<int32_t> goff_dev;
    reo::DevBuf<uint64_t> t_kin, t_kout;
    reo::DevBuf<uint16_t> t_vin, t_vout;
    reo::DevBuf<unsigned char> t_temp;
    reo::DevBuf<int32_t> t_order, t_flags, t_slots;
    reo::DevBuf<uint32_t> unit_map;
    std::vector<uint32_t> unit_map_host;
    std::vector<int32_t> t_order_host, t_slots_host, goff_blocks_host;
    const int32_t *t_meta_ptr[3] = {nullptr, nullptr, nullptr};
    int32_t *host_flags = nullptr;
    hipEvent_t ev_flags = nullptr;
    bool table_prezeroed = false;
    const uint32_t *unit_map_uploaded = nullptr;
    size_t k1_items_n = 0;
    bool transformed = false;
    int eager_mode = 2;
    int eager_chunk = 0;
    int eager_gate = 1;
    hipStream_t up = nullptr, rk = nullptr;
    hipEvent_t ev_up[8] = {nullptr};
    hipEvent_t ev_rk[4] = {nullptr, nullptr, nullptr, nullptr};
    reo::DevBuf<int32_t> e_lists;
    int upload_threads = 12;
    unsigned char *stage_h[3] = {nullptr, nullptr, nullptr};
    size_t stage_cap = 0;
    reo::DevBuf<unsigned char> stage_d[3];
    hipEvent_t ev_stage[3] = {nullptr, nullptr, nullptr}, ev_widen[3] = {nullptr, nullptr, nullptr};
    int64_t narrowed_bytes = 0;
    int rowmajor_upload = 0;
    int csc_upload = 0;
    int64_t csc_nnz = 0;
    reo::DevBuf<int64_t> csc_colptr;
    int csc_device = 0;
    bool eager_k1 = false;
    int has_ties = 0;
    int transform_in_lds = 0;

    reo::DevBuf<uint32_t> table;
    int built_k = -1;
    int built_treat = -1;
    bool table_complete = false;
    void *comm = nullptr;
    int spin_wait = 0;
    int check_hook_table = 1;
    bool comm_dead = false;
    bool in_multi = false;
    bool multi_one_device = false;
    std::vector<reo_ctx *> peers;
    reo::DevBuf<uint16_t> gcounts;
    bool gc_valid = false;
    int k1_wave = 1;
    int k1_order = 0;
    int k1_half = 1;
    int k1_slots = 1;
    int last_k1_slots = 0;
    int k1_unslot = -1;
    int k1_slot_sides = 0;
    int last_k1_slot_sides = 0;
    int last_k1_unslot = 0;
    int k1_unslot_attr = 0;
    const uint32_t *k1_slot_items = nullptr;
    size_t k1_slot_items_n = 0;
    int k1_slot_gp = 0;
    reo::DevBuf<uint32_t> k1_slot_part;
    reo::DevBuf<uint32_t> k1_slot_maps;
    reo::DevBuf<uint4> pos_s, lo_s;
    int k1_slot_slice = 1;
    int last_k1_slot_slice = 0;
    bool planes_ready = false;
    int planes_on_demand = 0;
    int k1_queue = 1;
    int k1_workers = 0;
    reo::DevBuf<uint32_t> k1_queue_ctr;
    int n_cus = 256;
    int share_counts = 1;
    int last_k1_shared = 0;
    int64_t tiles_owned = 0, tiles_total = 0;
    int k1_cj = 0, k1_q = 0;
    std::vector<uint32_t> units_all_host, units_all_dev;
    const uint32_t *units_all_uploaded = nullptr;
    reo::DevBuf<uint32_t> units_all, xsend, xrecv;
    int x_waves = 4;
    bool x_pipelined = false;
    hipStream_t k1s[2] = {nullptr, nullptr}, xs = nullptr;
    hipEvent_t ev_fork = nullptr, ev_k1[8] = {nullptr}, ev_k1_join[2] = {nullptr, nullptr}, ev_x = nullptr;
    struct ItemList { reo::DevBuf<uint32_t> buf; size_t n = 0; uint64_t key[5] = {0, 0, 0, 0, 0}; };
    ItemList k1_wave_items[8];
    reo::DevBuf<uint32_t> k1_park[2];
    reo::DevBuf<int32_t> k1_park_ge[2];
    int64_t eager_range_launches = 0;
    int eager_ranges = -1;
    reo::DevBuf<int32_t> check_flag;

    reo::DevBuf<uint32_t> refbits[2];
    reo::DevBuf<uint8_t> refbytes[2];
    int ref_slot = -1;
    const char *ref_gone = "reo_identify_degs has not run on this context";
    reo::DevBuf<int32_t> sc_slot2col;
    std::vector<int32_t> sc_slot2col_host;
    const int32_t *sc_slot2col_uploaded = nullptr;
    reo::DevBuf<double> st_lf;
    int64_t st_lf_G = -1;
    reo::DevBuf<uint8_t> vmask;
    bool vmask_set = false;
    int64_t vmask_G = 0, vmask_S = 0;
    reo::DevBuf<uint32_t> vwords;
    bool vwords_valid = false;
    reo::DevBuf<int32_t> mp_thr;
    std::vector<int32_t> mp_thr_host;
    int32_t mp_thr_n[2] = {-1, -1};
    double mp_thr_pval = -1.0;
    const int32_t *mp_thr_uploaded = nullptr;
    int built_masked = 0;
    int64_t perm_batch = 0;
    int64_t perm_kernel_us = 0;
    int64_t top_hist_us = 0;
    int64_t top_emit_us = 0;
    int64_t top_null_batch = 0;
    int64_t top_null_us = 0;
    reo::DevBuf<int32_t> raw;
    reo::DevBuf<uint32_t> delta_list;
    reo::DevBuf<int32_t> cont;
    reo::DevBuf<double> result;
    reo::DevBuf<double> sorted_d;
    reo::DevBuf<double> sorted_p;
    reo::DevBuf<uint32_t> rank_s, rank_a;
    reo::DevBuf<double> scal;
    reo::DevBuf<double> blockmin;
    reo::DevBuf<double> chunk_v;
    reo::DevBuf<uint16_t> chunk_i;
    reo::DevBuf<double> part;
    reo::DevBuf<reo::IterState> state;
    reo::DevBuf<int32_t> trace;
    reo::DevBuf<int32_t> modes;
    reo::DevBuf<double> cand;
    reo::DevBuf<unsigned> gridbar;
    reo::DevBuf<reo::LightState> lstate;
    reo::DevBuf<int32_t> clist;
    int light_band = 32;
    bool cycle_watch = true;
    reo::DevBuf<uint8_t> snap;
    int it_cycle_period = 0, it_cycle_at = 0, it_cycle_skipped = 0;
    int hist_below = 256;
    int xcc_local = 0;
    int light_window = 24, light_min_g = 4096;
    int light_mode = 1;
    reo::DevBuf<int32_t> olist;
    reo::DevBuf<int32_t> hist, mrank;
    double it_pval_deg = 1.0, it_padj_deg = 0.05;
    int it_n_iter = 0, it_n_conv = 0, it_a0 = 0, it_b0 = 0;
    int k2_idx = 0;
// ... 145 lines not shown
```

### rankcompv3.jl_amd/csrc/transform.hip

```cpp
#include <sched.h>
#include <cctype>
#include <cmath>
#include <cstdio>
#include <cstdlib>
#include <cstring>

#ifdef REO_WITH_ROCPRIM
#include <rocprim/rocprim.hpp>
#endif

#include <algorithm>
#include <chrono>
#include <atomic>
#include <condition_variable>
#include <functional>
#include <limits>
#include <mutex>
#include <numeric>
#include <thread>
#include <type_traits>

#include "reo_internal.h"
#include "upload_rows.h"
#include "upload_csc.h"
// ... 1045 lines not shown
    std::vector<int32_t> order(S);
    std::iota(order.begin(), order.end(), 0);
    std::stable_sort(order.begin(), order.end(),
                     [&](int a, int b) { return c->group_id[a] < c->group_id[b]; });
    c->goff.assign(c->ngroups + 1, 0);
    for (int s = 0; s < S; ++s) c->goff[c->group_id[s] + 1]++;
    for (int g = 0; g < c->ngroups; ++g) c->goff[g + 1] += c->goff[g];
    c->goff32.assign(c->ngroups + 1, 0);
    for (int g = 0; g < c->ngroups; ++g) c->goff32[g + 1] = c->goff32[g] + (c->goff[g + 1] - c->goff[g] + 31) / 32 * 32;
    const int S32 = c->goff32[c->ngroups], nblk = S32 / 32;
    std::vector<int32_t> slots(S), goff_blocks(c->ngroups + 1);
    for (int t = 0; t < S; ++t) {
        const int g = c->group_id[order[t]];
        slots[t] = c->goff32[g] + (t - c->goff[g]);
    }
    for (int g = 0; g < c->ngroups; ++g)
        for (int sl = c->goff32[g] + (c->goff[g + 1] - c->goff[g]); sl < c->goff32[g + 1]; ++sl) slots.push_back(sl);
    for (int g = 0; g <= c->ngroups; ++g) goff_blocks[g] = c->goff32[g] / 32;

    DevBuf<int32_t> &d_order = c->t_order, &d_flags = c->t_flags;
    int32_t rc;
    if ((rc = d_order.ensure(S)) || (rc = d_flags.ensure(32)) || (rc = c->t_slots.ensure(slots.size()))) return rc;
    if ((rc = c->goff_dev.ensure(c->ngroups + 1))) return rc;
    if (order != c->t_order_host || slots != c->t_slots_host || goff_blocks != c->goff_blocks_host || d_order.p != c->t_meta_ptr[0] ||
        c->t_slots.p != c->t_meta_ptr[1] || c->goff_dev.p != c->t_meta_ptr[2]) {
        REO_HIP_CHECK(hipMemcpyAsync(d_order.p, order.data(), sizeof(int32_t) * S, hipMemcpyHostToDevice, st));
        REO_HIP_CHECK(hipMemcpyAsync(c->t_slots.p, slots.data(), sizeof(int32_t) * slots.size(), hipMemcpyHostToDevice, st));
        REO_HIP_CHECK(hipMemcpyAsync(c->goff_dev.p, goff_blocks.data(), sizeof(int32_t) * (c->ngroups + 1),
                                     hipMemcpyHostToDevice, st));
        REO_HIP_CHECK(hipStreamSynchronize(st));
        c->t_order_host = order; c->t_slots_host = slots; c->goff_blocks_host = goff_blocks;
        c->t_meta_ptr[0] = d_order.p; c->t_meta_ptr[1] = c->t_slots.p; c->t_meta_ptr[2] = c->goff_dev.p;
    }
    REO_HIP_CHECK(hipMemsetAsync(d_flags.p, 0, 6 * sizeof(int32_t), st));
    unsigned long long *d_varbits = reinterpret_cast<unsigned long long *>(d_flags.p + 2);

    const bool big = G > 65535;
    const size_t n = static_cast<size_t>(S32) * Gp;
    const size_t nq = static_cast<size_t>(nblk) * Gp * 4;
    if (!big) {
        if ((rc = c->t_pos16.ensure(n)) || (rc = c->t_lo16.ensure(n)) || (rc = c->t_hi16.ensure(n)) ||
            (rc = c->pos.ensure(nq)) || (rc = c->lo.ensure(nq)) || (rc = c->hi.ensure(nq)))
            return rc;
    } else {
        if ((rc = c->t_pos32.ensure(n)) || (rc = c->t_lo32.ensure(n)) || (rc = c->t_hi32.ensure(n)) ||
            (rc = c->pos.ensure(static_cast<size_t>(nblk) * Gp * 5)) || (rc = c->lo.ensure(static_cast<size_t>(nblk) * Gp * 8)) ||
            (rc = c->hi.ensure(static_cast<size_t>(nblk) * Gp * 8)))
            return rc;
        REO_HIP_CHECK(hipMemsetAsync(c->t_pos32.p, 0, n * sizeof(uint32_t), st));
        REO_HIP_CHECK(hipMemsetAsync(c->t_lo32.p, 0, n * sizeof(uint32_t), st));
        REO_HIP_CHECK(hipMemsetAsync(c->t_hi32.p, 0, n * sizeof(uint32_t), st));
        REO_HIP_CHECK(hipMemsetAsync(c->lo.p, 0, static_cast<size_t>(nblk) * Gp * 8 * sizeof(uint4), st));
        REO_HIP_CHECK(hipMemsetAsync(c->hi.p, 0, static_cast<size_t>(nblk) * Gp * 8 * sizeof(uint4), st));
    }
    const T *X = static_cast<const T *>(c->dX);
    c->planes_ready = false; c->planes_on_demand = 0;
    auto slice = [&]() -> int32_t {
        if (big) t_slice_big<<<dim3(Gp / 256, nblk), 256, 0, st>>>(c->t_pos32.p, c->t_lo32.p, c->t_hi32.p, Gp, c->pos.p, c->lo.p, c->hi.p);
        else t_slice<<<dim3(Gp / 512, nblk), 256, 0, st>>>(c->t_pos16.p, c->t_lo16.p, c->t_hi16.p, Gp, c->pos.p, c->lo.p, c->hi.p, 0);
        REO_HIP_CHECK(hipGetLastError());
        c->planes_ready = true;
        return REO_OK;
    };
    auto finish = [&](int has_ties, bool sliced) -> int32_t {
        if (!sliced) { const int32_t rs = slice(); if (rs) return rs; }
        c->has_ties = has_ties;
        c->transformed = true;
        return REO_OK;
    };
    const bool planes_can_wait = c->k1_slots && c->k1_slot_slice && c->k1_wave && !big && S <= 65535 && c->ngroups == 2 && c->world == 1 && !c->in_multi;

    const char *env = getenv("REO_TRANSFORM");
    c->transform_in_lds = 0;
    if (G <= 65535 && !(env && env[0] == 's')) {
        if (!c->host_flags) REO_HIP_CHECK(pool_alloc(reinterpret_cast<void **>(&c->host_flags), 8 * sizeof(int32_t), true));
        if (!c->ev_flags) REO_HIP_CHECK(handle_event(&c->ev_flags, 0));
        int32_t *fl = c->host_flags;
        bool wide = !kCountingPath<T> || (env && env[0] == 'w');
        for (int attempt = 0; attempt < 2; ++attempt) {
            if ((rc = launch_lds_ranking<T>(c, X, SampleList{d_order.p, c->t_slots.p, S, S32}, d_flags.p, wide))) return rc;
            if (!planes_can_wait && (rc = slice())) return rc;
            REO_HIP_CHECK(hipMemcpyAsync(fl, d_flags.p, 6 * sizeof(int32_t), hipMemcpyDeviceToHost, st));
            REO_HIP_CHECK(hipEventRecord(c->ev_flags, st));
            if (!c->table_prezeroed && c->table.p && c->table.n >= static_cast<size_t>(c->G) * 4 * c->Wp) {
                REO_HIP_CHECK(hipMemsetAsync(c->table.p, 0, static_cast<size_t>(c->G) * 4 * c->Wp * sizeof(uint32_t), st));
                c->table_prezeroed = true;
            }
            REO_HIP_CHECK(hipEventSynchronize(c->ev_flags));
            if (fl[0]) {
                set_error(kNaNMessage);
                return REO_EINVAL;
            }
            if (c->debug_stamps && wide) {
                unsigned long long stv[8];
                REO_HIP_CHECK(hipMemcpy(stv, d_flags.p + 8, sizeof stv, hipMemcpyDeviceToHost));
                fprintf(stderr, "stamps t_sample_wide (max + flags, sample sort, histogram, prefix sums, scatter, ranks in slot order, into gene order + rows):");
                for (int k = 1; k <= 5; ++k) fprintf(stderr, " %lld", (long long)(stv[k] - stv[k - 1]));
                fprintf(stderr, " %lld %lld", (long long)(stv[7] - stv[5]), (long long)(stv[6] - stv[7]));
                fprintf(stderr, "  (x 10 ns)\n");
            }
            if (c->debug_stamps && !wide) {
                unsigned long long stv[6];
                REO_HIP_CHECK(hipMemcpy(stv, d_flags.p + 8, sizeof stv, hipMemcpyDeviceToHost));
                fprintf(stderr, "stamps t_sample, histogram form (column read + varying bits, clear, keys + histogram, prefix sums, rows out):");
                for (int k = 1; k <= 5; ++k) fprintf(stderr, " %lld", (long long)(stv[k] - stv[k - 1]));
                fprintf(stderr, "  (x 10 ns)\n");
            }
            if (!fl[4] && !fl[5]) {
                c->transform_in_lds = wide ? 2 : 1;
                if (planes_can_wait && fl[1] && (rc = slice())) return rc;
                return finish(fl[1], true);
            }
            REO_HIP_CHECK(hipMemsetAsync(d_flags.p, 0, 6 * sizeof(int32_t), st));
            if (wide) { set_error("the bucket form of the ranking flagged a sample: internal error"); return REO_EHIP; }
            wide = true;
        }
    }
    if (big && !(env && env[0] == 's')) {
        const size_t lds = 8 * (kSplit1 + 16) + 4 * (static_cast<size_t>(kSplit1) * 17 + 1 + ((static_cast<size_t>(kSplit1) * 17 + 1) >> 5) + 1 + 17) + 16;
        REO_HIP_CHECK(hipFuncSetAttribute(reinterpret_cast<const void *>(t_sample_big<T>), hipFuncAttributeMaxDynamicSharedMemorySize, 160 * 1024));
        const int batch = static_cast<int>(std::max<size_t>(1, std::min<size_t>(static_cast<size_t>(S), (size_t(4) << 30) / (static_cast<size_t>(Gp) * 8))));
        if ((rc = c->t_kin.ensure(static_cast<size_t>(batch) * Gp))) return rc;
        for (int s0 = 0; s0 < S; s0 += batch) {
            const int ns = std::min(batch, S - s0);
            t_sample_big<T><<<static_cast<unsigned>(ns), 1024, lds, st>>>(X, c->ld, d_order.p + s0, c->t_slots.p + s0, G, Gp, c->t_pos32.p, c->t_lo32.p, c->t_hi32.p,
                                                                      d_flags.p, c->t_kin.p);
            REO_HIP_CHECK(hipGetLastError());
        }
        if ((rc = slice())) return rc;
        int32_t flags[2] = {0, 0};
        REO_HIP_CHECK(hipMemcpyAsync(flags, d_flags.p, sizeof flags, hipMemcpyDeviceToHost, st));
        REO_HIP_CHECK(hipStreamSynchronize(st));
        if (flags[0]) {
            set_error(kNaNMessage);
            return REO_EINVAL;
        }
        c->transform_in_lds = 3;
        return finish(flags[1], true);
    }
#ifdef REO_WITH_ROCPRIM
    if (!big) {
        REO_HIP_CHECK(hipMemsetAsync(c->t_pos16.p, 0, n * sizeof(uint16_t), st));
        REO_HIP_CHECK(hipMemsetAsync(c->t_lo16.p, 0, n * sizeof(uint16_t), st));
        REO_HIP_CHECK(hipMemsetAsync(c->t_hi16.p, 0, n * sizeof(uint16_t), st));
    }

    const int CB = std::max(1, std::min(std::min(S, 65535), static_cast<int>((1u << 27) / static_cast<unsigned>(G))));
    DevBuf<uint64_t> &k_in = c->t_kin, &k_out = c->t_kout;
    const size_t bn = static_cast<size_t>(CB) * G;
    if ((rc = k_in.ensure(bn)) || (rc = k_out.ensure(bn))) return rc;
    auto seg_begin = rocprim::make_transform_iterator(rocprim::counting_iterator<unsigned>(0),
                                                      SegOff{static_cast<unsigned>(G)});
    auto segmented = [&](auto &v_in, auto &v_out, auto *pos, auto *lo, auto *hi) -> int32_t {
        using IdxT = std::remove_pointer_t<decltype(pos)>;
        int32_t rc2;
        if ((rc2 = v_in.ensure(bn)) || (rc2 = v_out.ensure(bn))) return rc2;
        size_t temp_bytes = 0;
        REO_HIP_CHECK(rocprim::segmented_radix_sort_pairs(nullptr, temp_bytes, k_in.p, k_out.p, v_in.p, v_out.p,
                                                          static_cast<unsigned>(bn), static_cast<unsigned>(CB),
                                                          seg_begin, seg_begin + 1, 0, 64, st));
        DevBuf<unsigned char> &temp = c->t_temp;
        if ((rc2 = temp.ensure(std::max<size_t>(temp_bytes, 16)))) return rc2;
        for (int cb0 = 0; cb0 < S; cb0 += CB) {
            const int nc = std::min(CB, S - cb0);
            dim3 grid((G + 255) / 256, nc);
            REO_HIP_CHECK(hipMemsetAsync(d_varbits, 0, sizeof(unsigned long long), st));
            t_keys<T, IdxT><<<grid, 256, 0, st>>>(X, c->ld, d_order.p, G, cb0, k_in.p, v_in.p, d_flags.p, d_varbits);
// ... 1058 lines not shown
```

Baseline: 52470 billion.

## Synthesize constant slot-separated table words in unslot instead of memset plus emit

```diff
diff --git a/rankcompv3.jl_amd/_ffi.py b/rankcompv3.jl_amd/_ffi.py
--- a/rankcompv3.jl_amd/_ffi.py
+++ b/rankcompv3.jl_amd/_ffi.py
@@ -1164,8 +1164,8 @@
                 "k2_full_launches": int(ms[9]), "k2_delta_ms": ms[10], "set_matrix_host_wall_ms": ms[11]}
 
     def info(self) -> dict:
-        w = np.zeros(40, dtype=np.int64)
-        check(self._L.reo_get_info(self._h, _ptr(w), 40))
+        w = np.zeros(42, dtype=np.int64)
+        check(self._L.reo_get_info(self._h, _ptr(w), 42))
         v = np.zeros(28, dtype=np.int64)
         v[:] = w[:28]
         return {"G": int(v[0]), "S": int(v[1]), "Gp": int(v[2]), "table_bytes": int(v[3]), "has_ties": int(v[4]),
@@ -1180,4 +1180,5 @@
                 "masked_build": int(w[31]), "k1_slot_slice": int(w[32]), "planes_on_demand": int(w[33]),
                 "perm_batch": int(w[34]), "perm_kernel_us": int(w[35]),
                 "top_pairs_hist_us": int(w[36]), "top_pairs_emit_us": int(w[37]),
-                "top_pairs_null_batch": int(w[38]), "top_pairs_null_us": int(w[39])}
+                "top_pairs_null_batch": int(w[38]), "top_pairs_null_us": int(w[39]),
+                "k1_table_synth": int(w[40]), "k1_table_clear_words": int(w[41])}
diff --git a/rankcompv3.jl_amd/csrc/api.hip b/rankcompv3.jl_amd/csrc/api.hip
--- a/rankcompv3.jl_amd/csrc/api.hip
+++ b/rankcompv3.jl_amd/csrc/api.hip
@@ -334,7 +334,7 @@
     c->eager_k1 = false;
     c->vwords_valid = false;
     (void)mask_in_force(c);
-    c->last_k1_slots = 0; c->last_k1_slot_sides = 0; c->k1_slot_items = nullptr; c->k1_slot_items_n = 0; c->k1_slot_gp = 0;
+    c->last_k1_slots = 0; c->last_k1_slot_sides = 0; c->last_k1_synth = 0; c->last_k1_clear_words = 0; c->k1_slot_items = nullptr; c->k1_slot_items_n = 0; c->k1_slot_gp = 0;
 }
 
 static size_t elem_bytes(int dtype) { return dtype >= 3 ? 4 : 8; }
@@ -619,6 +619,8 @@
     if (const char *e = getenv("REO_K1_UNSLOT")) { const int v = atoi(e); c->k1_unslot = (v == 8 || v == 4) ? v : (e[0] == '0' ? 0 : -1); }
     if (const char *e = getenv("REO_K1_SLOT_SIDES")) { const int v = atoi(e); c->k1_slot_sides = (v == 1 || v == 2) ? v : 0; }
     if (const char *e = getenv("REO_K1_SLOT_SLICE")) c->k1_slot_slice = atoi(e) != 0;
+    if (const char *e = getenv("REO_K1_SYNTH")) c->k1_synth = (e[0] != '0');
+    if (const char *e = getenv("REO_K1_POISON")) c->k1_poison = (e[0] == '1');
     if (const char *e = getenv("REO_K1_WORKERS")) c->k1_workers = std::max(1, atoi(e));
     if (const char *e = getenv("REO_K1_ORDER")) c->k1_order = std::max(0, std::min(2, atoi(e)));
     {
@@ -1193,9 +1195,9 @@
     if ((rc = ensure_valid_words(c, "reo_build_pairs_masked"))) return rc;
     drop_ref_mask(c, "reo_build_pairs_masked has replaced the class table that the last reo_identify_degs ran on: no reo_identify_degs has run on the current one");
     c->built_k = -1; c->built_treat = -1; c->built_masked = 0; c->eager_k1 = false; c->table_complete = false;
-    c->last_k1_slots = 0; c->last_k1_slot_sides = 0; c->k1_slot_items = nullptr; c->k1_slot_items_n = 0; c->k1_slot_gp = 0; c->last_k1_shared = 0;
+    c->last_k1_slots = 0; c->last_k1_slot_sides = 0; c->last_k1_synth = 0; c->last_k1_clear_words = 0; c->k1_slot_items = nullptr; c->k1_slot_items_n = 0; c->k1_slot_gp = 0; c->last_k1_shared = 0;
     REO_HIP_CHECK(hipMemsetAsync(c->table.p, 0, static_cast<size_t>(c->G) * kPlanes * c->Wp * sizeof(uint32_t), c->stream));
-    c->table_prezeroed = false;
+    c->table_prezeroed = false; c->table_synth_prev = false;
     if ((rc = launch_pairs_masked(c, k, c->mp_thr.p, n1, c->mp_thr.p + n1 + 1, n2, min_complete[0], min_complete[1]))) return rc;
     c->built_k = k; c->built_masked = 1; c->table_complete = true;
     return REO_OK;
@@ -1670,7 +1672,7 @@
         int32_t rc = use(c);
         if (rc || (rc = launch_slot_separated(c, &separated))) return rc;
     }
-    const int64_t v[40] = {c->G, c->S, c->Gp, static_cast<int64_t>(c->table.n * sizeof(uint32_t)), c->has_ties,
+    const int64_t v[42] = {c->G, c->S, c->Gp, static_cast<int64_t>(c->table.n * sizeof(uint32_t)), c->has_ties,
                            c->tiles_owned, c->tiles_total, kTileI, c->k1_cj, c->k1_q, kUnitH,
                            c->goff32.empty() ? 0 : c->goff32.back(), c->last_k1_shared,
                            static_cast<int64_t>(c->gcounts.n * sizeof(uint16_t)), c->transform_in_lds, c->xcc_local,
@@ -1679,9 +1681,10 @@
                            c->last_k1_slots ? c->last_k1_unslot : 0, c->built_k >= 0 ? c->built_treat : -1,
                            c->last_k1_slots ? c->last_k1_slot_sides : 0, (c->built_k >= 0 && c->built_masked) ? 1 : 0,
                            c->last_k1_slots ? c->last_k1_slot_slice : 0, c->transformed ? c->planes_on_demand : 0, c->perm_batch, c->perm_kernel_us,
-                           c->top_hist_us, c->top_emit_us, c->top_null_batch, c->top_null_us};
-    for (int i = 0; i < n && i < 40; ++i) info[i] = v[i];
-    return REO_OK;
-}
-
-}
+                           c->top_hist_us, c->top_emit_us, c->top_null_batch, c->top_null_us,
+                           c->last_k1_slots ? c->last_k1_synth : 0, c->last_k1_clear_words};
+    for (int i = 0; i < n && i < 42; ++i) info[i] = v[i];
+    return REO_OK;
+}
+
+}
diff --git a/rankcompv3.jl_amd/csrc/k1_slots.h b/rankcompv3.jl_amd/csrc/k1_slots.h
--- a/rankcompv3.jl_amd/csrc/k1_slots.h
+++ b/rankcompv3.jl_amd/csrc/k1_slots.h
@@ -234,6 +234,87 @@
         for (int c = 0; c < 32; ++c) ks[c] = g2s[32 * wo + c];
         unslot_out_word<R>(u, ks, wo, T, G, 32 * Wp);
         for (int q = 0; q < 2 * nr; ++q) rows[unslot_pair_word(q, side, Wp, wo)] = u[q];
+    }
+}
+
+constexpr int kSynthLoad = 4;
+
+REO_SLOTS_HD int slot_const_class(int n, int hi_thr, int lo_thr) { return n >= hi_thr ? 2 : (n <= lo_thr ? 1 : 0); }
+REO_SLOTS_HD int slot_synth_classes(int n_side, int hi_thr) { return slot_const_class(n_side, hi_thr, n_side - hi_thr) | slot_const_class(0, hi_thr, n_side - hi_thr) << 2; }
+
+REO_SLOTS_HD int slot_synth_word(int s, uint32_t row_trng, uint32_t row_crng, int w, uint32_t w_trng, uint32_t w_crng, int G, int classes)
+{
+    const int bw = w >> 1, bs = s >> 6;
+    const bool fwd = bw > bs;
+    const int sep = slot_separated(fwd ? row_trng : w_trng, fwd ? w_crng : row_crng);
+    const int cls = sep > 0 ? (classes & 3) : ((classes >> 2) & 3);
+    int v = (fwd || !cls) ? cls : 3 - cls;
+    v = (sep == 0 || bw == bs) ? kSynthLoad : v;
+    return 32 * w >= G ? 0 : v;
+}
+REO_SLOTS_HD uint32_t slot_synth_fill(int decision, int plane) { return ((decision >> plane) & 1) ? 0xFFFFFFFFu : 0u; }
+
+REO_SLOTS_HD size_t slot_synth_clear_words(int G) { return static_cast<size_t>(G) * 8; }
+
+inline void slot_diag_clear_model(uint32_t *table, int G, int Wp, const uint32_t *g2s, int side)
+{
+    for (int g = 0; g < G; ++g)
+        for (int p = 0; p < 2; ++p) {
+            uint32_t *row = table + (static_cast<size_t>(g) * 4 + 2 * side + p) * Wp + 2 * (g2s[g] >> 6);
+            row[0] = row[1] = 0u;
+        }
+}
+
+template <int R>
+inline void unslot_pair_synth_model(uint32_t *table, int r0, int n_rows, int side, int G, int Wp, const uint32_t *g2s, const uint32_t *trng, const uint32_t *crng,
+                                    int classes, uint32_t *T)
+{
+    const int nr = n_rows - r0 < 2 * R ? n_rows - r0 : 2 * R;
+    if (nr <= 0) return;
+    uint32_t *rows = table + static_cast<size_t>(r0) * 4 * Wp;
+    for (int w = 0; w < Wp; ++w) {
+        uint32_t m[4 * R];
+        for (int q = 0; q < 4 * R; ++q) {
+            m[q] = 0u;
+            if (q >= 2 * nr) continue;
+            const int s = static_cast<int>(g2s[r0 + (q >> 1)]);
+            const int d = slot_synth_word(s, trng[s >> 5], crng[s >> 8], w, trng[w], crng[w >> 3], G, classes);
+            m[q] = d == kSynthLoad ? rows[unslot_pair_word(q, side, Wp, w)] : slot_synth_fill(d, q & 1);
+        }
+        unslot_in_word<R>(m, w, T);
+    }
+    for (int wo = 0; wo < Wp; ++wo) {
+        uint32_t u[4 * R], ks[32];
+        for (int c = 0; c < 32; ++c) ks[c] = g2s[32 * wo + c];
+        unslot_out_word<R>(u, ks, wo, T, G, 32 * Wp);
+        for (int q = 0; q < 2 * nr; ++q) rows[unslot_pair_word(q, side, Wp, wo)] = u[q];
+    }
+}
+
+template <int R>
+inline void unslot_group_synth_model(uint32_t *table, int r0, int n_rows, int G, int Wp, const uint32_t *g2s, const uint32_t *trng, const uint32_t *crng,
+                                     const int *classes, uint32_t *T)
+{
+    const int nr = n_rows - r0 < R ? n_rows - r0 : R;
+    if (nr <= 0) return;
+    uint32_t *rows = table + static_cast<size_t>(r0) * 4 * Wp;
+    for (int w = 0; w < Wp; ++w) {
+        uint32_t m[4 * R];
+        for (int q = 0; q < 4 * R; ++q) {
+            m[q] = 0u;
+            if (q >= 4 * nr) continue;
+            const int s = static_cast<int>(g2s[r0 + (q >> 2)]), z = (q >> 1) & 1;
+            const uint32_t *tr = trng + static_cast<size_t>(z) * Wp, *cr = crng + static_cast<size_t>(z) * (Wp / 8);
+            const int d = slot_synth_word(s, tr[s >> 5], cr[s >> 8], w, tr[w], cr[w >> 3], G, classes[z]);
+            m[q] = d == kSynthLoad ? rows[static_cast<size_t>(q) * Wp + w] : slot_synth_fill(d, q & 1);
+        }
+        unslot_in_word<R>(m, w, T);
+    }
+    for (int wo = 0; wo < Wp; ++wo) {
+        uint32_t u[4 * R], ks[32];
+        for (int c = 0; c < 32; ++c) ks[c] = g2s[32 * wo + c];
+        unslot_out_word<R>(u, ks, wo, T, G, 32 * Wp);
+        for (int q = 0; q < 4 * nr; ++q) rows[static_cast<size_t>(q) * Wp + wo] = u[q];
     }
 }
 
diff --git a/rankcompv3.jl_amd/csrc/kernels.hip b/rankcompv3.jl_amd/csrc/kernels.hip
--- a/rankcompv3.jl_amd/csrc/kernels.hip
+++ b/rankcompv3.jl_amd/csrc/kernels.hip
@@ -181,6 +181,7 @@
     const uint32_t *trng, *crng;
     uint32_t *queue;
     uint32_t n_items;
+    int synth;
 };
 constexpr size_t kParkSlot = 2 * 64 * 64;
 
@@ -421,7 +422,7 @@
     int sep = 0;
     if constexpr (SLOTS) sep = __builtin_amdgcn_readfirstlane(slot_separated(a.trng[side * (a.Gp >> 5) + (i0 >> 5)], a.crng[side * (a.Gp >> 8) + (jw >> 8)]));
     if (SLOTS && sep) {
-        emit_constant<RI>(a, i0, jl, side, sep > 0 ? (side ? a.nt : a.nc) : 0);
+        if (!a.synth) emit_constant<RI>(a, i0, jl, side, sep > 0 ? (side ? a.nt : a.nc) : 0);
     } else if (be > bb) {
         const char *pb = reinterpret_cast<const char *>(a.P) + static_cast<size_t>(bb) * LQ * a.Gp * 16;
         const size_t aoff = (static_cast<size_t>(bb) * a.Gp + i0) * ROWB;
@@ -646,7 +647,7 @@
     if (n) atomicAdd(&g2s[g], n);
 }
 
-__global__ __launch_bounds__(256) void k1_slot_invert(uint32_t *__restrict__ g2s, uint32_t *__restrict__ s2g, int G, int Gp, int sides)
+__global__ __launch_bounds__(256) void k1_slot_invert(uint32_t *__restrict__ g2s, uint32_t *__restrict__ s2g, int G, int Gp, int sides, uint32_t *__restrict__ diag)
 {
     const int g = blockIdx.x * 256 + threadIdx.x;
     if (g >= Gp) return;
@@ -656,6 +657,10 @@
     else g2s[g] = v;
     s2g[k] = v;
     if (sides != 2) s2g[static_cast<size_t>(Gp) + k] = v;
+    if (diag && g < G) {
+        const int Wp = Gp >> 5, p0 = sides == 2 ? 2 * static_cast<int>(blockIdx.y) : 0, p1 = sides == 2 ? p0 + 2 : kPlanes;
+        for (int p = p0; p < p1; ++p) *reinterpret_cast<uint2 *>(diag + (static_cast<size_t>(g) * kPlanes + p) * Wp + 2 * (k >> 6)) = uint2{0u, 0u};
+    }
 }
 
 __global__ __launch_bounds__(256) void k1_slot_ranges(const uint32_t *__restrict__ gmm, const uint32_t *__restrict__ s2g, int G, int Gp,
@@ -752,8 +757,13 @@
     }
 }
 
-template <int R>
-__global__ __launch_bounds__(kUnslotThreadsMax) void k1_unslot_words(uint32_t *__restrict__ table, const uint32_t *__restrict__ g2s, int G, int Wp)
+struct UnslotSynth {
+    const uint32_t *trng, *crng;
+    int classes[2];
+};
+
+template <int R, bool SYNTH = false>
+__global__ __launch_bounds__(kUnslotThreadsMax) void k1_unslot_words(uint32_t *__restrict__ table, const uint32_t *__restrict__ g2s, int G, int Wp, UnslotSynth sy)
 {
     constexpr int NQ = 4 * R;
     extern __shared__ uint32_t unslot_t[];
@@ -761,10 +771,39 @@
     if (nr <= 0) return;
     const int nq = nr * kPlanes;
     uint32_t *rows = table + static_cast<size_t>(r0) * kPlanes * Wp;
+    int rs[SYNTH ? R : 1];
+    uint32_t rt[SYNTH ? 2 * R : 1], rc[SYNTH ? 2 * R : 1];
+    if constexpr (SYNTH) {
+        static_assert(R <= 64, "a lane per row");
+        const int lane = static_cast<int>(threadIdx.x & 63u);
+        const uint32_t vs = min(g2s[min(r0 + min(lane, R - 1), G - 1)], static_cast<uint32_t>(32 * Wp - 1));
+        const uint32_t vt0 = sy.trng[vs >> 5], vt1 = sy.trng[Wp + (vs >> 5)], vc0 = sy.crng[vs >> 8], vc1 = sy.crng[(Wp >> 3) + (vs >> 8)];
+#pragma unroll
+        for (int r = 0; r < R; ++r) {
+            rs[r] = __builtin_amdgcn_readlane(static_cast<int>(vs), r);
+            rt[2 * r] = static_cast<uint32_t>(__builtin_amdgcn_readlane(static_cast<int>(vt0), r)); rt[2 * r + 1] = static_cast<uint32_t>(__builtin_amdgcn_readlane(static_cast<int>(vt1), r));
+            rc[2 * r] = static_cast<uint32_t>(__builtin_amdgcn_readlane(static_cast<int>(vc0), r)); rc[2 * r + 1] = static_cast<uint32_t>(__builtin_amdgcn_readlane(static_cast<int>(vc1), r));
+        }
+    }
     for (int w = threadIdx.x; w < Wp; w += blockDim.x) {
         uint32_t m[NQ];
-#pragma unroll
-        for (int q = 0; q < NQ; ++q) m[q] = q < nq ? rows[static_cast<size_t>(q) * Wp + w] : 0u;
+        if constexpr (SYNTH) {
+#pragma unroll
+            for (int z = 0; z < 2; ++z) {
+                const uint32_t *tr = sy.trng + static_cast<size_t>(z) * Wp, *cr = sy.crng + static_cast<size_t>(z) * (Wp >> 3);
+                const uint32_t wt = tr[w], wc = cr[w >> 3];
+#pragma unroll
+                for (int r = 0; r < R; ++r) {
+                    const int q = 4 * r + 2 * z;
+                    const int d = r < nr ? slot_synth_word(rs[r], rt[2 * r + z], rc[2 * r + z], w, wt, wc, G, sy.classes[z]) : 0;
+                    m[q] = slot_synth_fill(d, 0); m[q + 1] = slot_synth_fill(d, 1);
+                    if (d == kSynthLoad) { m[q] = rows[static_cast<size_t>(q) * Wp + w]; m[q + 1] = rows[static_cast<size_t>(q + 1) * Wp + w]; }
+                }
+            }
+        } else {
+#pragma unroll
+            for (int q = 0; q < NQ; ++q) m[q] = q < nq ? rows[static_cast<size_t>(q) * Wp + w] : 0u;
+        }
         unslot_in_word<R>(m, w, unslot_t);
     }
     __syncthreads();
@@ -783,8 +822,8 @@
     }
 }
 
-template <int R>
-__global__ __launch_bounds__(kUnslotThreadsMax) void k1_unslot_pair(uint32_t *__restrict__ table, const uint32_t *__restrict__ g2s, int G, int Wp)
+template <int R, bool SYNTH = false>
+__global__ __launch_bounds__(kUnslotThreadsMax) void k1_unslot_pair(uint32_t *__restrict__ table, const uint32_t *__restrict__ g2s, int G, int Wp, UnslotSynth sy)
 {
     constexpr int NQ = 4 * R;
     extern __shared__ uint32_t unslot_t[];
@@ -793,10 +832,36 @@
     const int nq = nr * 2;
     g2s += static_cast<size_t>(side) * 32 * Wp;
     uint32_t *rows = table + static_cast<size_t>(r0) * kPlanes * Wp;
+    const uint32_t *tr = sy.trng + static_cast<size_t>(side) * Wp, *cr = sy.crng + static_cast<size_t>(side) * (Wp >> 3);
+    int rs[SYNTH ? 2 * R : 1];
+    uint32_t rt[SYNTH ? 2 * R : 1], rc[SYNTH ? 2 * R : 1];
+    if constexpr (SYNTH) {
+        const int lane = static_cast<int>(threadIdx.x & 63u);
+        const uint32_t vs = min(g2s[min(r0 + min(lane, 2 * R - 1), G - 1)], static_cast<uint32_t>(32 * Wp - 1));
+        const uint32_t vt = tr[vs >> 5], vc = cr[vs >> 8];
+#pragma unroll
+        for (int r = 0; r < 2 * R; ++r) {
+            rs[r] = __builtin_amdgcn_readlane(static_cast<int>(vs), r);
+            rt[r] = static_cast<uint32_t>(__builtin_amdgcn_readlane(static_cast<int>(vt), r));
+            rc[r] = static_cast<uint32_t>(__builtin_amdgcn_readlane(static_cast<int>(vc), r));
+        }
+    }
     for (int w = threadIdx.x; w < Wp; w += blockDim.x) {
         uint32_t m[NQ];
-#pragma unroll
-        for (int q = 0; q < NQ; ++q) m[q] = q < nq ? rows[unslot_pair_word(q, side, Wp, w)] : 0u;
+        if constexpr (SYNTH) {
+            const uint32_t wt = tr[w], wc = cr[w >> 3];
+            const int classes = side ? sy.classes[1] : sy.classes[0];
+#pragma unroll
+            for (int r = 0; r < 2 * R; ++r) {
+                const int q = 2 * r;
+                const int d = r < nr ? slot_synth_word(rs[r], rt[r], rc[r], w, wt, wc, G, classes) : 0;
+                m[q] = slot_synth_fill(d, 0); m[q + 1] = slot_synth_fill(d, 1);
+                if (d == kSynthLoad) { m[q] = rows[unslot_pair_word(q, side, Wp, w)]; m[q + 1] = rows[unslot_pair_word(q + 1, side, Wp, w)]; }
+            }
+        } else {
+#pragma unroll
+            for (int q = 0; q < NQ; ++q) m[q] = q < nq ? rows[unslot_pair_word(q, side, Wp, w)] : 0u;
+        }
         unslot_in_word<R>(m, w, unslot_t);
     }
     __syncthreads();
@@ -3713,7 +3778,8 @@
         if ((rc = item_list(c, a, pl, 3, wunits[w], c->k1_wave_items[w], w, nwaves))) return rc;
     if ((rc = upload_units_all(c))) return rc;
     if (!c->table_prezeroed) REO_HIP_CHECK(hipMemsetAsync(c->table.p, 0, static_cast<size_t>(c->G) * kPlanes * c->Wp * sizeof(uint32_t), c->stream));
-    c->table_prezeroed = false;
+    c->table_prezeroed = false; c->table_synth_prev = false;
+    c->last_k1_clear_words = static_cast<int64_t>(c->G) * kPlanes * c->Wp;
     c->last_k1_shared = 0;
     tic(c, 1);
     int32_t xrc = REO_OK;
@@ -3818,6 +3884,7 @@
     a.park = nullptr; a.park_ge = nullptr; a.park_mode = 0;
     a.s2g = nullptr; a.trng = nullptr; a.crng = nullptr;
     a.queue = nullptr; a.n_items = 0;
+    a.synth = 0;
     return a;
 }
 
@@ -3898,7 +3965,7 @@
         k1_slot_sort<false><<<dim3(spans, zs), kSlotRankSpan / 2, 0, c->stream>>>(m.key, G, Gp, m.srt);
         k1_slot_rank<false><<<dim3(gb, spans, zs), 256, 0, c->stream>>>(m.key, m.srt, G, Gp, m.g2s);
     }
-    k1_slot_invert<<<dim3(static_cast<unsigned>(Gp / 256), zs), 256, 0, c->stream>>>(m.g2s, m.s2g, G, Gp, sides);
+    k1_slot_invert<<<dim3(static_cast<unsigned>(Gp / 256), zs), 256, 0, c->stream>>>(m.g2s, m.s2g, G, Gp, sides, a.synth ? a.table : nullptr);
     k1_slot_ranges<<<dim3(static_cast<unsigned>(Gp / 256), 2), 256, 0, c->stream>>>(m.gmm, m.s2g, G, Gp, m.trng, m.crng);
     if (c->k1_slot_slice) {
         const int per = (nblk * (Gp / 512) + 7) / 8;
@@ -3926,22 +3993,26 @@
         if ((c->k1_unslot == kUnslotWide || c->k1_unslot == kUnslotNarrow) && unslot_lds_bytes(c->k1_unslot, a.Gp) <= kUnslotLdsLimit) form = c->k1_unslot;
         const size_t lds = unslot_lds_bytes(form, a.Gp);
         if (lds <= kUnslotLdsLimit) {
-            auto go = [&](auto rtag) -> int32_t {
+            auto go = [&](auto rtag, auto stag) -> int32_t {
                 constexpr int R = decltype(rtag)::value;
-                const int bit = (R == kUnslotWide ? 1 : 2) << (sides == 2 ? 2 : 0);
-                const void *fn = sides == 2 ? reinterpret_cast<const void *>(k1_unslot_pair<R>) : reinterpret_cast<const void *>(k1_unslot_words<R>);
+                constexpr bool S = decltype(stag)::value;
+                const int bit = (R == kUnslotWide ? 1 : 2) << ((sides == 2 ? 2 : 0) + (S ? 4 : 0));
+                const void *fn = sides == 2 ? reinterpret_cast<const void *>(k1_unslot_pair<R, S>) : reinterpret_cast<const void *>(k1_unslot_words<R, S>);
                 if (!(c->k1_unslot_attr & bit)) {
                     REO_HIP_CHECK(hipFuncSetAttribute(fn, hipFuncAttributeMaxDynamicSharedMemorySize, static_cast<int>(kUnslotLdsLimit)));
                     c->k1_unslot_attr |= bit;
                 }
                 const unsigned threads = static_cast<unsigned>(unslot_threads(a.Wp));
+                const UnslotSynth sy{a.trng, a.crng, {slot_synth_classes(a.nc, a.m1), slot_synth_classes(a.nt, a.m2)}};
                 if (sides == 2)
-                    k1_unslot_pair<R><<<dim3(static_cast<unsigned>((a.G + 2 * R - 1) / (2 * R)), 2), threads, lds, c->stream>>>(a.table, slot_maps(c).g2s, a.G, a.Wp);
+                    k1_unslot_pair<R, S><<<dim3(static_cast<unsigned>((a.G + 2 * R - 1) / (2 * R)), 2), threads, lds, c->stream>>>(a.table, slot_maps(c).g2s, a.G, a.Wp, sy);
                 else
-                    k1_unslot_words<R><<<static_cast<unsigned>((a.G + R - 1) / R), threads, lds, c->stream>>>(a.table, slot_maps(c).g2s, a.G, a.Wp);
+                    k1_unslot_words<R, S><<<static_cast<unsigned>((a.G + R - 1) / R), threads, lds, c->stream>>>(a.table, slot_maps(c).g2s, a.G, a.Wp, sy);
                 return REO_OK;
             };
-            const int32_t rc = form == kUnslotWide ? go(std::integral_constant<int, kUnslotWide>{}) : go(std::integral_constant<int, kUnslotNarrow>{});
+            int32_t rc;
+            if (a.synth) rc = form == kUnslotWide ? go(std::integral_constant<int, kUnslotWide>{}, std::true_type{}) : go(std::integral_constant<int, kUnslotNarrow>{}, std::true_type{});
+            else rc = form == kUnslotWide ? go(std::integral_constant<int, kUnslotWide>{}, std::false_type{}) : go(std::integral_constant<int, kUnslotNarrow>{}, std::false_type{});
             if (rc) return rc;
             REO_HIP_CHECK(hipGetLastError());
             c->last_k1_unslot = form;
@@ -4002,7 +4073,7 @@
     if ((rc = upload_unit_map(c, units))) return rc;
     a.unit_map = c->unit_map.p;
     a.gate = gate;
-    if (!prepare) { c->last_k1_slots = 0; c->last_k1_slot_sides = 0; c->last_k1_slot_slice = 0; c->k1_slot_items = nullptr; c->k1_slot_items_n = 0; c->k1_slot_gp = 0; }
+    if (!prepare) { c->last_k1_slots = 0; c->last_k1_slot_sides = 0; c->last_k1_slot_slice = 0; c->last_k1_synth = 0; c->last_k1_clear_words = 0; c->k1_slot_items = nullptr; c->k1_slot_items_n = 0; c->k1_slot_gp = 0; }
     if ((range || prepare) && (sides != 1 && sides != 2)) { set_error("a range of sample blocks / a prepared launch: one side of the pair kernel"); return REO_EINVAL; }
     if (gate && (!pl.wave || pl.wide || pl.big)) { set_error("a gated launch of the pair kernel: wave form, at most 65535 genes and samples"); return REO_EINVAL; }
     c->x_pipelined = false;
@@ -4027,16 +4098,25 @@
         if (range && (rc = apply_range(c, a, sides, range, il.n))) return rc;
         if (c->k1_stamps) REO_HIP_CHECK(hipMalloc(reinterpret_cast<void **>(&a.stamps), (std::max<size_t>(c->k1_items_n, 1) * 4 + 2) * sizeof(unsigned long long)));
     }
-    if (!keep_table) {
-        if (!c->table_prezeroed) REO_HIP_CHECK(hipMemsetAsync(c->table.p, 0, static_cast<size_t>(c->G) * kPlanes * c->Wp * sizeof(uint32_t), c->stream));
+    if (!units.empty() && k1_slots_wanted(c, pl, sides, keep_table, gate, range, prepare) && c->k1_items_n) {
+        if (k1_slots_alloc(c) == REO_OK) pl.slots = true;
+        else (void)hipGetLastError();
+    }
+    a.synth = (pl.slots && c->k1_synth && c->k1_unslot != 0 && unslot_lds_bytes(kUnslotNarrow, a.Gp) <= kUnslotLdsLimit) ? 1 : 0;
+    const size_t table_bytes = static_cast<size_t>(c->G) * kPlanes * c->Wp * sizeof(uint32_t);
+    if (a.synth) {
+        c->last_k1_clear_words = static_cast<int64_t>(c->table_prezeroed ? table_bytes / sizeof(uint32_t) : slot_synth_clear_words(c->G));
+        if (c->k1_poison) REO_HIP_CHECK(hipMemsetAsync(c->table.p, 0xFF, table_bytes, c->stream));
         c->table_prezeroed = false;
-    }
+    } else if (!keep_table) {
+        if (!c->table_prezeroed) REO_HIP_CHECK(hipMemsetAsync(c->table.p, 0, table_bytes, c->stream));
+        c->table_prezeroed = false;
+        c->last_k1_clear_words = static_cast<int64_t>(table_bytes / sizeof(uint32_t));
+    }
+    c->last_k1_synth = a.synth;
+    c->table_synth_prev = a.synth != 0;
     if (units.empty()) return REO_OK;
     c->last_k1_shared = pl.shared ? 1 : 0;
-    if (k1_slots_wanted(c, pl, sides, keep_table, gate, range, prepare) && c->k1_items_n) {
-        if (k1_slots_alloc(c) == REO_OK) pl.slots = true;
-        else (void)hipGetLastError();
-    }
     if (!(pl.slots && c->k1_slot_slice) && (rc = ensure_planes(c))) return rc;
     if (a.stamps) k_time_mark<<<1, 64, 0, c->stream>>>(a.stamps + c->k1_items_n * 4);
     tic(c, 1);
diff --git a/rankcompv3.jl_amd/csrc/reo_internal.h b/rankcompv3.jl_amd/csrc/reo_internal.h
--- a/rankcompv3.jl_amd/csrc/reo_internal.h
+++ b/rankcompv3.jl_amd/csrc/reo_internal.h
@@ -241,6 +241,11 @@
     reo::DevBuf<uint4> pos_s, lo_s;
     int k1_slot_slice = 1;
     int last_k1_slot_slice = 0;
+    int k1_synth = 1;
+    int k1_poison = 0;
+    int last_k1_synth = 0;
+    int64_t last_k1_clear_words = 0;
+    bool table_synth_prev = false;
     bool planes_ready = false;
     int planes_on_demand = 0;
     int k1_queue = 1;
diff --git a/rankcompv3.jl_amd/csrc/transform.hip b/rankcompv3.jl_amd/csrc/transform.hip
--- a/rankcompv3.jl_amd/csrc/transform.hip
+++ b/rankcompv3.jl_amd/csrc/transform.hip
@@ -1151,7 +1151,7 @@
             if (!planes_can_wait && (rc = slice())) return rc;
             REO_HIP_CHECK(hipMemcpyAsync(fl, d_flags.p, 6 * sizeof(int32_t), hipMemcpyDeviceToHost, st));
             REO_HIP_CHECK(hipEventRecord(c->ev_flags, st));
-            if (!c->table_prezeroed && c->table.p && c->table.n >= static_cast<size_t>(c->G) * 4 * c->Wp) {
+            if (!c->table_prezeroed && !c->table_synth_prev && c->table.p && c->table.n >= static_cast<size_t>(c->G) * 4 * c->Wp) {
                 REO_HIP_CHECK(hipMemsetAsync(c->table.p, 0, static_cast<size_t>(c->G) * 4 * c->Wp * sizeof(uint32_t), st));
                 c->table_prezeroed = true;
             }
```

Result: no change. 52660 billion, median of 5 (+0.4%).
